# mimoralea/gym-soccer-littman94

Hardware: AMD Instinct MI355X
Metric: env-steps/sec (whole node) at batch=1M random joint actions; HBM GB/s vs peak (higher is better)
Workload: dtype int8

## Files before the change

gym_soccer_littman94_amd/csrc/soccer_handle.hpp:

```cpp
#pragma once
#include <hip/hip_runtime.h>

#include <string>
#include <vector>

#include "../../include/soccer_hip.h"
#include "soccer_inlists.hpp"
#include "soccer_kernels.hpp"
#include "soccer_plan_io.hpp"
#include "soccer_rules.hpp"

#pragma GCC visibility push(hidden)

using namespace soccer;

int fail(soccer_handle* h, int code, const char* fmt, ...);

#define HIP_TRY(h, expr)                                                                         \
    do {                                                                                         \
        hipError_t e_ = (expr);                                                                  \
        if (e_ != hipSuccess)                                                                    \
            return fail((h), e_ == hipErrorOutOfMemory ? SOCCER_E_NOMEM : SOCCER_E_HIP,          \
                        "%s failed: %s", #expr, hipGetErrorString(e_));                          \
    } while (0)

template <typename T>
static inline bool aligned(const T* p, size_t a) { return p == nullptr || (reinterpret_cast<uintptr_t>(p) % a) == 0; }

template <class T> static inline T* off(T* p, unsigned long long lanes) { return p ? p + lanes : nullptr; }

struct OwnedBufs {
    struct Buf { void* ptr; bool pinned; };
    enum PinnedFlags : unsigned { kPinned = hipHostMallocDefault, kPinnedMapped = hipHostMallocMapped };
    const char* what;
    std::vector<Buf> bufs;
    bool ready = false;
    explicit OwnedBufs(const char* owner) : what(owner) {}
    OwnedBufs(const OwnedBufs&) = delete;
    OwnedBufs& operator=(const OwnedBufs&) = delete;
    ~OwnedBufs() { clear(); }

    template <class T>
    int alloc(soccer_handle* h, size_t count, T** out) { return take(h, hipMalloc(out, bytes<T>(count)), false, out); }
    template <class T>
    int alloc_pinned(soccer_handle* h, size_t count, PinnedFlags flags, T** out) { return take(h, hipHostMalloc(out, bytes<T>(count), flags), true, out); }
    template <class T>
    int upload(soccer_handle* h, const std::vector<T>& v, const T** out) {
        T* d = nullptr;
        if (int rc = alloc(h, v.size(), &d)) return rc;
        if (!v.empty() && hipMemcpy(d, v.data(), v.size() * sizeof(T), hipMemcpyHostToDevice) != hipSuccess)
            return fail(h, SOCCER_E_HIP, "upload of %s failed", what);
        *out = d;
        return SOCCER_OK;
    }
    void release(void* p) {
        for (size_t i = 0; i < bufs.size(); ++i) if (bufs[i].ptr == p) { drop(bufs[i]); bufs.erase(bufs.begin() + i); return; }
    }
    void clear() {
        for (const Buf& b : bufs) drop(b);
        bufs.clear(); ready = false;
    }

private:
    template <class T> static size_t bytes(size_t count) { return count ? count * sizeof(T) : 1; }
    static void drop(const Buf& b) { (void)(b.pinned ? hipHostFree(b.ptr) : hipFree(b.ptr)); }
    template <class T>
    int take(soccer_handle* h, hipError_t e, bool pinned, T** out) {
        if (e != hipSuccess) {
            *out = nullptr;
            return e == hipErrorOutOfMemory ? fail(h, SOCCER_E_NOMEM, "out of %s memory for %s", pinned ? "pinned host" : "device", what)
                                            : fail(h, SOCCER_E_HIP, "allocation for %s failed: %s", what, hipGetErrorString(e));
        }
        bufs.push_back(Buf{*out, pinned});
        return SOCCER_OK;
    }
};

struct soccer_graph {
    hipGraph_t graph = nullptr;
    hipGraphExec_t exec = nullptr;
    uint64_t ticks = 0;
    int start_slot = 0;
    bool stamped = false;
    int32_t kernel_nodes = 0;
    int64_t steps_fused = 0;
    int32_t fused_launches = 0;
};

struct PendingRun {
    soccer_step_args first{};
    int64_t len = 0;
    int64_t act_stride = 0, out_stride = 0;
};

struct Learner;

struct soccer_handle {
    soccer_config cfg{};
    Rules rules;
    KernelParams P{};
    hipStream_t stream = nullptr;
    bool own_stream = false;
    hipEvent_t ev0 = nullptr, ev1 = nullptr;
    OwnedBufs bufs{"the handle"};
    uint16_t* d_lut = nullptr; uint32_t* d_nc = nullptr; uint32_t* d_isd = nullptr;
    int8_t* d_policy[2] = {nullptr, nullptr};
    unsigned long long* d_tick = nullptr;
    unsigned long long* d_hist = nullptr;
    unsigned int* d_misuse = nullptr;
    unsigned int* misuse_host = nullptr;
    uint8_t* d_state = nullptr;
    size_t state_stride = 0;
    int state_streams = 6;
    uint8_t* stage_dev = nullptr;
    uint8_t* stage_host = nullptr;
    bool mapped = false;
    size_t stage_bytes = 0;
    int tick_slot = 0;
    uint64_t tick = 0;
    bool slip = false, lut_lds = false;
    size_t smem_bytes = 0;
    int E = 4;
    int grid_cap = 2048;
    bool capturing = false;
    uint64_t capture_ticks = 0;
    int capture_calls = 0;
    int capture_start_slot = 0;
    PendingRun run;
    bool graph_fuse = true;
    int capture_kernels = 0;
    int64_t capture_steps_fused = 0; int capture_fused_launches = 0;
    unsigned long long* d_hist_unread = nullptr;
    int n_cu = 256;
    size_t lds_limit = 64 * 1024;
    uint4* d_sub = nullptr;
    uint4* rec_host = nullptr; uint4* rec_dev = nullptr; uint32_t rec_seq = 0;
    swar::Consts swar_c{}; bool swar_ok = false;
    swar::SlipConsts slip_c{}; bool slip_swar_ok = false;
    uint32_t* d_slip_lut = nullptr;
    uint32_t* d_slip_step_lut = nullptr;
    size_t hist_slots = kHistSlots;
    bool timer_stamped = false; int wall_clock_khz = 100000;
    bool capture_stamped = false;
    bool stamp_poll = false;
    unsigned long long stamp_prev = 0;
    unsigned long long swar_launch_lanes = kSwarLaunchLanes;
    int rollout_pref = 0;
    soccer_rollout_shape_info last_rollout{};
    SlipF64* d_slip_f64 = nullptr;
    uint32_t* d_worklist = nullptr;
    unsigned long long* d_traj_hist = nullptr;
    void* comm = nullptr; int comm_world = 0, comm_rank = 0;
    unsigned long long* d_comm_scratch = nullptr;
    PlanIO plan{};
    OwnedBufs plan_bufs{"the planner lists"};
    MinimaxIO mm{};
    double* mm_V[2] = {nullptr, nullptr};
    unsigned long long* mm_words = nullptr;
    OwnedBufs mm_bufs{"the minimax planner"};
    double* br_pol[2] = {nullptr, nullptr};
    double* br_V[2] = {nullptr, nullptr};
    double* br_Qr = nullptr;
    int32_t* br_arg = nullptr;
    unsigned long long* br_words = nullptr;
    int br_cap = 0; bool br_pairs = false;
    OwnedBufs br_bufs{"the best-response solver"};
    double* cx_pol = nullptr;
    double* cx_V[2] = {nullptr, nullptr};
    unsigned long long* cx_words = nullptr;
    int32_t* cx_done = nullptr;
    int32_t* cx_iter = nullptr;
    double* cx_payoff = nullptr;
    int32_t* cx_open = nullptr;
    double* cx_values = nullptr;
    int cx_policies = 0, cx_stride = 0; bool cx_has_values = false;
    OwnedBufs cx_bufs{"the cross-play solver"};
    double* mo_pol = nullptr;
    double* mo_V[2] = {nullptr, nullptr};
    unsigned long long* mo_words = nullptr;
    int32_t* mo_done = nullptr;
    int32_t* mo_iter = nullptr;
    double* mo_kickoff = nullptr;
    int32_t* mo_open = nullptr;
    double* mo_values = nullptr;
    int mo_policies = 0, mo_stride = 0; bool mo_has_values = false;
    OwnedBufs mo_bufs{"the match-outcome solver"};
    const int32_t* oc_in_offset = nullptr;
    const InEntry* oc_in_list = nullptr;
    OwnedBufs oc_lists{"the occupancy solver's in-lists"};
    double* oc_pol = nullptr;
    double* oc_polT = nullptr;
    double* oc_D[2] = {nullptr, nullptr};
    unsigned long long* oc_words = nullptr;
    int32_t* oc_done = nullptr;
    int32_t* oc_iter = nullptr;
    double* oc_length = nullptr;
    double* oc_expect = nullptr;
    double* oc_features = nullptr;
    int32_t* oc_open = nullptr;
    double* oc_values = nullptr;
    int oc_policies = 0, oc_stride = 0; bool oc_has_values = false;
    OwnedBufs oc_bufs{"the occupancy solver"};
    double* pg_pol = nullptr;
    double* pg_polT = nullptr;
    double* pg_V[2] = {nullptr, nullptr};
    double* pg_D[2] = {nullptr, nullptr};
    double* pg_Q = nullptr;
    unsigned long long* pg_words = nullptr;
    int32_t* pg_done[2] = {nullptr, nullptr};
    int32_t* pg_iter = nullptr;
    double* pg_payoff = nullptr;
    int32_t* pg_open = nullptr;
    double* pg_grad = nullptr;
    double* pg_reach = nullptr;
    double* pg_w = nullptr;
    double* pg_values = nullptr;
    int pg_policies = 0, pg_stride = 0; bool pg_has_values = false;
    OwnedBufs pg_bufs{"the policy-gradient solver"};
    std::vector<soccer_gradient_play*> gradient_players;
    double* mg_A = nullptr;
    double* mg_T = nullptr;
    double* mg_x = nullptr; double* mg_y = nullptr;
    double* mg_fcol = nullptr; double* mg_prow = nullptr;
    int32_t* mg_basis = nullptr;
    double* mg_scal = nullptr;
    int32_t* mg_int = nullptr;
    size_t mg_need[5] = {0, 0, 0, 0, 0};
    OwnedBufs mg_bufs{"the meta-game solver"};
    std::vector<Learner*> learners;
    std::string err;

    soccer_handle() = default;
    soccer_handle(const soccer_handle&) = delete;
    soccer_handle& operator=(const soccer_handle&) = delete;
    ~soccer_handle();
};

constexpr size_t kStampStride = 8;
constexpr size_t kMappedBytes = 64 + 8 * kStampStride * SOCCER_STAMP_SLOTS;

static inline void bind_tick(soccer_handle* h, KernelParams& P, uint64_t ticks) {
    P.tick_in = h->d_tick + (h->tick_slot ? 16 : 0);
    P.tick_out = h->d_tick + (h->tick_slot ? 0 : 16);
    h->tick_slot ^= 1;
    if (h->capturing) { h->capture_ticks += ticks; h->capture_calls += 1; }
    else h->tick += ticks;
}

static inline void note_kernel(soccer_handle* h) { if (h->capturing) h->capture_kernels += 1; }

static inline int grid_for(const soccer_handle* h, uint64_t work_items) {
    uint64_t blocks = (work_items + kBlock - 1) / kBlock;
    if (blocks < 1) blocks = 1;
    if (blocks > (uint64_t)h->grid_cap) blocks = h->grid_cap;
    return static_cast<int>(blocks);
}

hipError_t rollout_raise_smem_limit(const soccer_handle* h, size_t bytes);
bool rollout_takes_swar(const soccer_handle* h, const soccer_rollout_args* a, const soccer_rollout_extra* x);
int rollout_enqueue(soccer_handle* h, const soccer_rollout_args* a, const soccer_rollout_extra* x, unsigned long long* hist);
int flush_run(soccer_handle* h);
static inline int flush_pending(soccer_handle* h) { return h->run.len ? flush_run(h) : SOCCER_OK; }
void comm_release(soccer_handle* h);
void learners_release(soccer_handle* h);
void gradient_players_release(soccer_handle* h);

#pragma GCC visibility pop
```

gym_soccer_littman94_amd/csrc/soccer_hip.hip:

```cpp
#include <hip/hip_runtime.h>

#include <algorithm>
#include <atomic>
#include <chrono>
#include <cstdarg>
#include <cstdio>
#include <cstdlib>
#include <cstring>
#include <memory>
#include <string>
#include <vector>

#include "soccer_handle.hpp"
#include "soccer_env_kernels.hpp"
#include "soccer_slip.hpp"

static thread_local std::string g_err;

int fail(soccer_handle* h, int code, const char* fmt, ...) {
    char buf[512];
    va_list ap; va_start(ap, fmt); vsnprintf(buf, sizeof buf, fmt, ap); va_end(ap);
    if (h) h->err = buf; else g_err = buf;
    return code;
}

extern "C" int soccer_abi_version(void) { return SOCCER_ABI_VERSION; }

extern "C" int soccer_device_count(int* count) {
    if (!count) return fail(nullptr, SOCCER_E_INVALID, "count is NULL");
    HIP_TRY(nullptr, hipGetDeviceCount(count));
    return SOCCER_OK;
}

extern "C" const char* soccer_last_error(const soccer_handle* h) { return h ? h->err.c_str() : g_err.c_str(); }

soccer_handle::~soccer_handle() {
    (void)hipSetDevice(cfg.device);
    (void)hipStreamSynchronize(stream);
    comm_release(this);
    learners_release(this);
    gradient_players_release(this);
    bufs.clear(); plan_bufs.clear(); mm_bufs.clear(); br_bufs.clear();
    if (ev0) (void)hipEventDestroy(ev0);
    if (ev1) (void)hipEventDestroy(ev1);
    if (own_stream && stream) (void)hipStreamDestroy(stream);
}

static void set_key(soccer_handle* h, uint64_t seed) {
    h->cfg.seed = seed;
    h->P.key0 = static_cast<uint32_t>(seed);
    h->P.key1 = static_cast<uint32_t>(seed >> 32);
}

extern "C" int soccer_create(const soccer_config* cfg, soccer_handle** out) {
    if (!cfg || !out) return fail(nullptr, SOCCER_E_INVALID, "cfg/out is NULL");
    *out = nullptr;
    if (cfg->n_lanes < 1) return fail(nullptr, SOCCER_E_INVALID, "n_lanes must be >= 1");
    if (!(cfg->slip_prob >= 0.0 && cfg->slip_prob <= 1.0))
        return fail(nullptr, SOCCER_E_INVALID, "slip_prob must be in [0, 1]");
    if (cfg->max_steps < 1 || cfg->max_steps > 250)
        return fail(nullptr, SOCCER_E_INVALID, "max_steps must be in 1..250 (timestep is a uint8)");
    const uint32_t e = cfg->envs_per_thread;
    if (!(e == 0 || e == 1 || e == 4 || e == 8))
        return fail(nullptr, SOCCER_E_INVALID, "envs_per_thread must be 0, 1, 4 or 8");
    std::unique_ptr<soccer_handle> owner(new soccer_handle());
    soccer_handle* h = owner.get();
    h->cfg = *cfg;
    const std::string msg = h->rules.build(cfg->width, cfg->height);
    if (!msg.empty()) return fail(nullptr, SOCCER_E_INVALID, "%s", msg.c_str());
    int ndev = 0;
    hipError_t de = hipGetDeviceCount(&ndev);
    if (de != hipSuccess || ndev < 1)
        return fail(nullptr, SOCCER_E_HIP, "no HIP device available (%s); libsoccer_hip has no CPU path",
                    de == hipSuccess ? "device count is 0" : hipGetErrorString(de));
    if (cfg->device < 0 || cfg->device >= ndev) return fail(nullptr, SOCCER_E_INVALID, "device %d out of range (0..%d)", cfg->device, ndev - 1);
    HIP_TRY(nullptr, hipSetDevice(cfg->device));
    if (cfg->flags & SOCCER_F_NULL_STREAM) { h->stream = nullptr; h->own_stream = false; }
    else if (cfg->stream) { h->stream = static_cast<hipStream_t>(cfg->stream); h->own_stream = false; }
    else { HIP_TRY(nullptr, hipStreamCreateWithFlags(&h->stream, hipStreamNonBlocking)); h->own_stream = true; }
    HIP_TRY(nullptr, hipEventCreate(&h->ev0));
    HIP_TRY(nullptr, hipEventCreate(&h->ev1));

    const Rules& R = h->rules;
    KernelParams& P = h->P;
    const size_t n = cfg->n_lanes;
    const size_t padded = (n + 255) & ~size_t(255);
    h->state_stride = padded;
    h->mapped = (cfg->flags & SOCCER_F_HOST_MAPPED) != 0;
    if (h->mapped && n > 4096) return fail(nullptr, SOCCER_E_INVALID, "SOCCER_F_HOST_MAPPED is for small handles (n_lanes <= 4096)");
    const char* lay = std::getenv("SOCCER_STATE_LAYOUT");
    const bool packed = swar::packs(R.H, R.W) && !h->mapped && !(lay && std::strcmp(lay, "wide") == 0);
    h->state_streams = packed ? 3 : 6;
    const size_t state_bytes = (size_t)h->state_streams * padded;
    if (int rc = h->mapped ? h->bufs.alloc_pinned(nullptr, state_bytes, OwnedBufs::kPinnedMapped, &h->d_state)
                           : h->bufs.alloc(nullptr, state_bytes, &h->d_state)) return rc;
    P.state = h->d_state; P.state_stride = padded; P.state_layout = packed ? kStatePacked : kStateWide;
    {
        uint8_t init[6] = {(uint8_t)R.isd[0][0], (uint8_t)R.isd[0][1], (uint8_t)R.isd[0][2], (uint8_t)R.isd[0][3], (uint8_t)(2 | R.isd[0][4]), 0};
        if (packed) {
            uint32_t a, b, t;
            swar::pack3(swar::Group{init[0], init[1], init[2], init[3], init[4], init[5]}, a, b, t);
            init[0] = (uint8_t)a; init[1] = (uint8_t)b; init[2] = (uint8_t)t;
        }
        for (int k = 0; k < h->state_streams; ++k) {
            if (h->mapped) std::memset(h->d_state + k * padded, init[k], padded);
            else HIP_TRY(nullptr, hipMemsetAsync(h->d_state + k * padded, init[k], padded, h->stream));
        }
    }

    if (int rc = h->bufs.alloc(nullptr, R.next_cell.size(), &h->d_nc)) return rc;
    if (int rc = h->bufs.alloc(nullptr, sizeof(R.isd_words) / sizeof(uint32_t), &h->d_isd)) return rc;
    HIP_TRY(nullptr, hipMemcpy(h->d_isd, R.isd_words, sizeof(R.isd_words), hipMemcpyHostToDevice));
    HIP_TRY(nullptr, hipMemcpy(h->d_nc, R.next_cell.data(), R.next_cell.size() * sizeof(uint32_t), hipMemcpyHostToDevice));
    if (int rc = h->bufs.alloc(nullptr, 256 / sizeof(unsigned long long), &h->d_tick)) return rc;
    HIP_TRY(nullptr, hipMemset(h->d_tick, 0, 256));
    while (h->hist_slots < (n + 255) / 256) h->hist_slots <<= 1;
    if (int rc = h->bufs.alloc(nullptr, h->hist_slots * kHistStride, &h->d_hist)) return rc;
    HIP_TRY(nullptr, hipMemset(h->d_hist, 0, sizeof(unsigned long long) * h->hist_slots * kHistStride));
    if (int rc = h->bufs.alloc(nullptr, h->hist_slots * kHistStride, &h->d_hist_unread)) return rc;
    HIP_TRY(nullptr, hipMemset(h->d_hist_unread, 0, sizeof(unsigned long long) * h->hist_slots * kHistStride));
    if (int rc = h->bufs.alloc_pinned(nullptr, kMappedBytes / sizeof(unsigned int), OwnedBufs::kPinnedMapped, &h->misuse_host)) return rc;
    std::memset(h->misuse_host, 0, kMappedBytes);
    HIP_TRY(nullptr, hipHostGetDevicePointer(reinterpret_cast<void**>(&h->d_misuse), h->misuse_host, 0));

    P.next_cell = h->d_nc; P.isd = h->d_isd;
    P.hist = h->d_hist; P.hist_mask = (uint32_t)(h->hist_slots - 1); P.misuse = h->d_misuse;
    P.lane_offset = cfg->lane_offset;
    P.first = 0; P.n = n; P.W = R.W; P.HW = R.H * R.W; P.HW5 = 5 * R.H * R.W;
    P.nc_len = static_cast<int32_t>(R.next_cell.size());
    P.max_steps = cfg->max_steps;
    P.autoreset = (cfg->flags & SOCCER_F_AUTORESET) ? 1u : 0u;
    P.step_stats = (cfg->flags & SOCCER_F_STEP_STATS) ? 1u : 0u;
    P.isd_shift = R.n_isd == 4 ? 0u : 1u;
    {
        const SlipTables ST = build_slip_tables(cfg->slip_prob);
        for (int i = 0; i < 4; ++i) P.w[i] = ST.w[i];
        for (int i = 0; i < 9; ++i) { P.B[i] = ST.B[i]; P.CB[i] = ST.CB[i]; }
        P.nb = ST.nb; P.act_pack = ST.act_pack; P.slip_int = ST.slip_int;
        static_assert(sizeof(swar::Quad) == sizeof(uint4), "threshold rows are 16 bytes");
        if (int rc = h->bufs.alloc(nullptr, sizeof(ST.sub) / sizeof(uint4), &h->d_sub)) return rc;
        HIP_TRY(nullptr, hipMemcpy(h->d_sub, ST.sub, sizeof(ST.sub), hipMemcpyHostToDevice));
        P.sub = h->d_sub;
        h->slip_swar_ok = ST.swar_ok;
        static_assert(kSlipBuckets == 16384 && kSlipThresholds == 40, "table layout shared with the kernels");
        if (ST.lut_ok) {
            std::vector<uint32_t> img(kSlipLdsWords, 0xFFFFFFFFu);
            std::memcpy(img.data(), ST.lut, kSlipBuckets);
            std::memcpy(img.data() + kSlipBuckets / 4, ST.T, sizeof(ST.T));
            if (int rc = h->bufs.alloc(nullptr, img.size(), &h->d_slip_lut)) return rc;
            HIP_TRY(nullptr, hipMemcpy(h->d_slip_lut, img.data(), img.size() * sizeof(uint32_t), hipMemcpyHostToDevice));
        }
        if (ST.lut_step_ok && !std::getenv("SOCCER_STEP_SLIP_ONE_BY_ONE")) {
            std::vector<uint32_t> img(kSlipStepLdsWords, 0xFFFFFFFFu);
            std::memcpy(img.data(), ST.lut_step, kSlipStepBuckets);
            std::memcpy(img.data() + kSlipStepBuckets / 4, ST.T, sizeof(ST.T));
            if (int rc = h->bufs.alloc(nullptr, img.size(), &h->d_slip_step_lut)) return rc;
            HIP_TRY(nullptr, hipMemcpy(h->d_slip_step_lut, img.data(), img.size() * sizeof(uint32_t), hipMemcpyHostToDevice));
        }
        {
            const SlipF64 F = make_slip_f64(ST);
            if (int rc = h->bufs.alloc(nullptr, 1, &h->d_slip_f64)) return rc;
            HIP_TRY(nullptr, hipMemcpy(h->d_slip_f64, &F, sizeof F, hipMemcpyHostToDevice));
        }
        h->slip_c = swar::SlipConsts{};
        for (int i = 0; i < 9; ++i) h->slip_c.CB[i] = ST.CB[i];
        h->slip_c.c_off = ST.c_off;
    }
    set_key(h, cfg->seed);
    h->swar_ok = swar::fits(R.H, R.W, cfg->max_steps);
    if (h->swar_ok) h->swar_c = swar::make_consts(R.H, R.W, R.goal_lo, R.goal_hi, cfg->max_steps, R.n_isd, R.isd, P.autoreset != 0u);
    h->slip = cfg->slip_prob != 0.0;
    if (const char* e2 = std::getenv("SOCCER_ROLLOUT")) h->rollout_pref = std::atoi(e2);
    if (const char* e4 = std::getenv("SOCCER_GRAPH_FUSE")) h->graph_fuse = std::atoi(e4) != 0;
    if (const char* e3 = std::getenv("SOCCER_SWAR_LAUNCH_LANES")) {
        const unsigned long long v = std::strtoull(e3, nullptr, 10) & ~3ull;
        if (v >= 4ull && v <= kSwarLaunchLanes) h->swar_launch_lanes = v;
    }
    h->E = e ? static_cast<int>(e) : 4;

    const size_t nc_bytes = (R.next_cell.size() + kIsdWords) * sizeof(uint32_t);
    const size_t lut_bytes = R.lut.size() * sizeof(uint16_t);
    if (nc_bytes > 150 * 1024)
        return fail(nullptr, SOCCER_E_INVALID, "pitch too large: the move/bounds table (%zu bytes) must fit the 160 KB LDS", nc_bytes);
    if (int rc = h->bufs.alloc(nullptr, R.lut.size(), &h->d_lut)) return rc;
    HIP_TRY(nullptr, hipMemcpy(h->d_lut, R.lut.data(), lut_bytes, hipMemcpyHostToDevice));
    P.lut = h->d_lut; P.lut_len = static_cast<int32_t>(R.lut.size());
    h->lut_lds = nc_bytes + lut_bytes <= 150 * 1024;
    h->smem_bytes = nc_bytes + (h->lut_lds ? lut_bytes : 0);
    if (h->smem_bytes > 48 * 1024) {
        const size_t b = h->smem_bytes;
        hipError_t se = rollout_raise_smem_limit(h, b);
        if (se == hipSuccess)
            se = hipFuncSetAttribute(h->slip ? reinterpret_cast<const void*>(h->lut_lds ? &reset_kernel<true, true> : &reset_kernel<false, true>)
                                             : reinterpret_cast<const void*>(h->lut_lds ? &reset_kernel<true, false> : &reset_kernel<false, false>),
                                     hipFuncAttributeMaxDynamicSharedMemorySize, (int)b);
        HIP_TRY(nullptr, se);
    }
    hipDeviceProp_t prop;
    HIP_TRY(nullptr, hipGetDeviceProperties(&prop, cfg->device));
    { int khz = 0; if (hipDeviceGetAttribute(&khz, hipDeviceAttributeWallClockRate, cfg->device) == hipSuccess && khz > 0) h->wall_clock_khz = khz; }
    h->grid_cap = prop.multiProcessorCount * 8;
    h->n_cu = prop.multiProcessorCount;
    if (prop.sharedMemPerBlockOptin > 0) h->lds_limit = prop.sharedMemPerBlockOptin;
    else if (prop.sharedMemPerBlock > 0) h->lds_limit = prop.sharedMemPerBlock;
    HIP_TRY(nullptr, hipStreamSynchronize(h->stream));
    HIP_TRY(nullptr, hipDeviceSynchronize());
    *out = owner.release();
    return SOCCER_OK;
}

extern "C" int soccer_destroy(soccer_handle* h) {
    delete h;
    return SOCCER_OK;
}

extern "C" int soccer_sync(soccer_handle* h) {
    if (!h) return fail(nullptr, SOCCER_E_INVALID, "handle is NULL");
    if (h->capturing) return fail(h, SOCCER_E_STATE, "soccer_sync during graph capture");
    HIP_TRY(h, hipSetDevice(h->cfg.device));
    HIP_TRY(h, hipStreamSynchronize(h->stream));
    return SOCCER_OK;
}

extern "C" int soccer_seed(soccer_handle* h, uint64_t seed) {
    if (!h) return fail(nullptr, SOCCER_E_INVALID, "handle is NULL");
    if (h->capturing) return fail(h, SOCCER_E_STATE, "soccer_seed during graph capture");
    HIP_TRY(h, hipSetDevice(h->cfg.device));
    set_key(h, seed);
    h->tick = 0;
    HIP_TRY(h, hipMemsetAsync(h->d_tick, 0, 256, h->stream));
    return SOCCER_OK;
}

extern "C" uint64_t soccer_tick(const soccer_handle* h) { return h ? h->tick : 0; }

extern "C" int soccer_set_tick(soccer_handle* h, uint64_t tick) {
    if (!h) return fail(nullptr, SOCCER_E_INVALID, "handle is NULL");
    if (h->capturing) return fail(h, SOCCER_E_STATE, "soccer_set_tick during graph capture");
    if (tick >> 63) return fail(h, SOCCER_E_INVALID, "tick must be below 2^63");
    HIP_TRY(h, hipSetDevice(h->cfg.device));
    HIP_TRY(h, hipStreamSynchronize(h->stream));
    unsigned long long slots[32] = {0};
    slots[0] = tick; slots[16] = tick;
    HIP_TRY(h, hipMemcpy(h->d_tick, slots, sizeof slots, hipMemcpyHostToDevice));
    h->tick = tick;
    return SOCCER_OK;
}
extern "C" uint64_t soccer_get_seed(const soccer_handle* h) { return h ? h->cfg.seed : 0; }

extern "C" int batched_reset(soccer_handle* h, const uint8_t* mask, const double* u_reset, uint16_t* obs) {
    if (!h) return fail(nullptr, SOCCER_E_INVALID, "handle is NULL");
    if (!aligned(u_reset, 8) || !aligned(obs, 2))
        return fail(h, SOCCER_E_INVALID, "batched_reset: u_reset must be 8-byte and obs 2-byte aligned");
    HIP_TRY(h, hipSetDevice(h->cfg.device));
    if (int rc = flush_pending(h)) return rc;
    KernelParams P = h->P;
    bind_tick(h, P, 1);
    ResetIO io{mask, u_reset, obs};
    unsigned long long n4 = 0;
    if (h->swar_ok && !u_reset && h->E != 1 && (P.lane_offset & 3ull) == 0ull && aligned(mask, 4) && aligned(obs, 8)) n4 = P.n & ~3ull;
    if (n4) {
        ResetSwar RS{h->swar_c, P.state, P.state_stride, P.state_layout, n4, P.lane_offset, P.tick_in, P.tick_out, P.key0, P.key1, mask, obs};
        const dim3 g(static_cast<unsigned>(((n4 >> 2) + kBlock - 1) / kBlock)), b(kBlock);
        if (h->slip) { if (mask) hipLaunchKernelGGL((reset_kernel_swar<true, true>), g, b, 0, h->stream, RS);
                       else hipLaunchKernelGGL((reset_kernel_swar<false, true>), g, b, 0, h->stream, RS); }
        else { if (mask) hipLaunchKernelGGL((reset_kernel_swar<true, false>), g, b, 0, h->stream, RS);
               else hipLaunchKernelGGL((reset_kernel_swar<false, false>), g, b, 0, h->stream, RS); }
        note_kernel(h);
    }
    if (n4 < P.n) {
        KernelParams Q = P;
        Q.first = n4; Q.n = P.n - n4;
        if (n4) Q.tick_out = nullptr;
        const int grid = grid_for(h, Q.n);
        if (h->slip) { if (h->lut_lds) hipLaunchKernelGGL((reset_kernel<true, true>), dim3(grid), dim3(kBlock), h->smem_bytes, h->stream, Q, io);
                       else hipLaunchKernelGGL((reset_kernel<false, true>), dim3(grid), dim3(kBlock), h->smem_bytes, h->stream, Q, io); }
        else { if (h->lut_lds) hipLaunchKernelGGL((reset_kernel<true, false>), dim3(grid), dim3(kBlock), h->smem_bytes, h->stream, Q, io);
               else hipLaunchKernelGGL((reset_kernel<false, false>), dim3(grid), dim3(kBlock), h->smem_bytes, h->stream, Q, io); }
        note_kernel(h);
    }
    HIP_TRY(h, hipGetLastError());
    return SOCCER_OK;
}

static int fetch_state(soccer_handle* h, std::vector<uint8_t>& img) {
    const size_t n = h->P.n, S = h->state_stride, bytes = (size_t)h->state_streams * S;
    if (h->mapped) std::memcpy(img.data(), h->d_state, bytes);
    else HIP_TRY(h, hipMemcpy(img.data(), h->d_state, bytes, hipMemcpyDeviceToHost));
    if (h->state_streams == 3) {
        for (size_t i = 0; i < n; ++i) {
            swar::Group G;
            swar::unpack3(img[i], img[S + i], img[2 * S + i], G);
            img[5 * S + i] = (uint8_t)G.tt; img[4 * S + i] = (uint8_t)G.ps; img[3 * S + i] = (uint8_t)G.cb;
            img[2 * S + i] = (uint8_t)G.rb; img[S + i] = (uint8_t)G.ca; img[i] = (uint8_t)G.ra;
        }
    }
    return SOCCER_OK;
}

extern "C" int soccer_state_streams(const soccer_handle* h) { return h ? h->state_streams : 0; }

extern "C" int soccer_set_state(soccer_handle* h, const int8_t* row_a, const int8_t* col_a, const int8_t* row_b,
                                const int8_t* col_b, const uint8_t* poss, const uint8_t* t,
                                const uint8_t* needs_reset) {
    if (!h) return fail(nullptr, SOCCER_E_INVALID, "handle is NULL");
    if (h->capturing) return fail(h, SOCCER_E_STATE, "soccer_set_state during graph capture");
    HIP_TRY(h, hipSetDevice(h->cfg.device));
    HIP_TRY(h, hipStreamSynchronize(h->stream));
    const size_t n = h->P.n, S = h->state_stride;
    const Rules& R = h->rules;
    std::vector<uint8_t> img(6 * S);
    if (int rc = fetch_state(h, img)) return rc;
    int8_t* ra = reinterpret_cast<int8_t*>(img.data());
    int8_t* ca = ra + S; int8_t* rb = ra + 2 * S; int8_t* cb = ra + 3 * S;
    uint8_t* ps = img.data() + 4 * S; uint8_t* tt = img.data() + 5 * S;
    for (size_t i = 0; i < n; ++i) {
        if (row_a) ra[i] = row_a[i];
        if (col_a) ca[i] = col_a[i];
        if (row_b) rb[i] = row_b[i];
        if (col_b) cb[i] = col_b[i];
        uint8_t p = ps[i] & 1, nr = (ps[i] >> 1) & 1;
        if (poss) { if (poss[i] > 1) return fail(h, SOCCER_E_INVALID, "lane %zu: possession must be 0 or 1", i); p = poss[i]; }
        if (needs_reset) nr = needs_reset[i] ? 1 : 0;
        ps[i] = static_cast<uint8_t>(p | (nr << 1));
        if (t) { if (t[i] > h->cfg.max_steps) return fail(h, SOCCER_E_INVALID, "lane %zu: timestep %d > max_steps", i, (int)t[i]); tt[i] = t[i]; }
        const bool in_range = ra[i] >= 0 && ra[i] < R.H && rb[i] >= 0 && rb[i] < R.H &&
                              ca[i] >= 0 && ca[i] < R.W && cb[i] >= 0 && cb[i] < R.W;
        if (!in_range || R.kind[R.flat(ra[i], ca[i], rb[i], cb[i], p)] == 0)
            return fail(h, SOCCER_E_INVALID, "lane %zu: state (%d, %d, %d, %d, %d) is not a reachable state tuple",
                        i, (int)ra[i], (int)ca[i], (int)rb[i], (int)cb[i], (int)p);
    }
    if (h->state_streams == 3) {
        for (size_t i = 0; i < n; ++i) {
            uint32_t a, b, t_;
            swar::pack3(swar::Group{(uint8_t)ra[i], (uint8_t)ca[i], (uint8_t)rb[i], (uint8_t)cb[i], ps[i], tt[i]}, a, b, t_);
            img[i] = (uint8_t)a; img[S + i] = (uint8_t)b; img[2 * S + i] = (uint8_t)t_;
        }
    }
    const size_t bytes = (size_t)h->state_streams * S;
    if (h->mapped) std::memcpy(h->d_state, img.data(), bytes);
    else HIP_TRY(h, hipMemcpy(h->d_state, img.data(), bytes, hipMemcpyHostToDevice));
    return SOCCER_OK;
}

extern "C" int soccer_host_view(soccer_handle* h, uint8_t** state, uint64_t* stride) {
    if (!h || !state || !stride) return fail(h, SOCCER_E_INVALID, "handle/state/stride is NULL");
    if (!h->mapped) return fail(h, SOCCER_E_STATE, "soccer_host_view needs a SOCCER_F_HOST_MAPPED handle");
    *state = h->d_state; *stride = h->state_stride;
    return SOCCER_OK;
}

extern "C" int soccer_get_state(soccer_handle* h, int8_t* row_a, int8_t* col_a, int8_t* row_b, int8_t* col_b,
                                uint8_t* poss, uint8_t* t, uint8_t* needs_reset) {
    if (!h) return fail(nullptr, SOCCER_E_INVALID, "handle is NULL");
    if (h->capturing) return fail(h, SOCCER_E_STATE, "soccer_get_state during graph capture");
    HIP_TRY(h, hipSetDevice(h->cfg.device));
    HIP_TRY(h, hipStreamSynchronize(h->stream));
    const size_t n = h->P.n, S = h->state_stride;
    std::vector<uint8_t> img(6 * S);
    if (int rc = fetch_state(h, img)) return rc;
    if (row_a) std::memcpy(row_a, img.data(), n);
    if (col_a) std::memcpy(col_a, img.data() + S, n);
    if (row_b) std::memcpy(row_b, img.data() + 2 * S, n);
    if (col_b) std::memcpy(col_b, img.data() + 3 * S, n);
    if (t) std::memcpy(t, img.data() + 5 * S, n);
    const uint8_t* ps = img.data() + 4 * S;
    for (size_t i = 0; i < n; ++i) {
        if (poss) poss[i] = ps[i] & 1;
        if (needs_reset) needs_reset[i] = (ps[i] >> 1) & 1;
    }
    return SOCCER_OK;
}

namespace {
struct StageLayout {
    size_t act_a, act_b, mask, u_step, u_reset;
    size_t obs, final_obs, reward, term, trunc, code;
    size_t out_begin, total;
};
StageLayout stage_layout(size_t n) {
    auto up = [](size_t x) { return (x + 63) & ~size_t(63); };
    StageLayout L{};
    size_t o = 0;
    L.act_a = o; o = up(o + n);
    L.act_b = o; o = up(o + n);
    L.mask = o; o = up(o + n);
    L.u_step = o; o = up(o + 8 * n);
    L.u_reset = o; o = up(o + 8 * n);
    L.out_begin = o;
    L.obs = o; o = up(o + 2 * n);
    L.final_obs = o; o = up(o + 2 * n);
    L.reward = o; o = up(o + n);
    L.term = o; o = up(o + n);
    L.trunc = o; o = up(o + n);
    L.code = o; o = up(o + n);
    L.total = o;
    return L;
}
int ensure_stage(soccer_handle* h, const StageLayout& L) {
    if (h->stage_bytes >= L.total) return SOCCER_OK;
    uint8_t* host = nullptr; uint8_t* dev = nullptr;
    if (int rc = h->bufs.alloc_pinned(h, L.total, h->mapped ? OwnedBufs::kPinnedMapped : OwnedBufs::kPinned, &host)) return rc;
    if (h->mapped) dev = host;
    else if (int rc = h->bufs.alloc(h, L.total, &dev)) { h->bufs.release(host); return rc; }
    h->stage_host = host; h->stage_dev = dev; h->stage_bytes = L.total;
    return SOCCER_OK;
}
}

extern "C" int soccer_staging(soccer_handle* h, soccer_staging_view* v) {
    if (!h || !v) return fail(h, SOCCER_E_INVALID, "handle/view is NULL");
    HIP_TRY(h, hipSetDevice(h->cfg.device));
    const StageLayout L = stage_layout(h->P.n);
    if (int rc = ensure_stage(h, L)) return rc;
    uint8_t* H = h->stage_host;
    v->act_a = reinterpret_cast<int8_t*>(H + L.act_a); v->act_b = reinterpret_cast<int8_t*>(H + L.act_b);
    v->mask = H + L.mask;
    v->u_step = reinterpret_cast<double*>(H + L.u_step); v->u_reset = reinterpret_cast<double*>(H + L.u_reset);
    v->obs = reinterpret_cast<uint16_t*>(H + L.obs); v->final_obs = reinterpret_cast<uint16_t*>(H + L.final_obs);
    v->reward = reinterpret_cast<int8_t*>(H + L.reward); v->terminated = H + L.term; v->truncated = H + L.trunc;
    v->prob_code = H + L.code;
    return SOCCER_OK;
}

static long first_bad_action(const int8_t* a, size_t n) {
    size_t i = 0;
    for (; i + 8 <= n; i += 8) {
        uint64_t v; std::memcpy(&v, a + i, 8);
        if ((v & 0xF8F8F8F8F8F8F8F8ull) | (((v & 0x0707070707070707ull) + 0x0303030303030303ull) & 0x0808080808080808ull)) break;
    }
    for (; i < n; ++i) if (a[i] < 0 || a[i] > 4) return (long)i;
    return -1;
}

extern "C" int batched_step_staged(soccer_handle* h, uint32_t use) {
    if (!h) return fail(nullptr, SOCCER_E_INVALID, "handle is NULL");
    if (h->capturing) return fail(h, SOCCER_E_STATE, "batched_step_staged during graph capture");
    const bool has_a = use & SOCCER_STAGE_ACT_A, has_b = use & SOCCER_STAGE_ACT_B;
    if ((!has_a && !h->P.policy_a) || (!has_b && !h->P.policy_b))
        return fail(h, SOCCER_E_INVALID, "batched_step: an action stream is required for every player without a fixed policy");
    HIP_TRY(h, hipSetDevice(h->cfg.device));
    const size_t n = h->P.n;
    const StageLayout L = stage_layout(n);
    if (int rc = ensure_stage(h, L)) return rc;
    uint8_t* H = h->stage_host; uint8_t* D = h->stage_dev;
    for (int pl = 0; pl < 2; ++pl) {
        if (!(pl ? has_b : has_a)) continue;
        const long bad = first_bad_action(reinterpret_cast<const int8_t*>(H + (pl ? L.act_b : L.act_a)), n);
        if (bad >= 0) return fail(h, SOCCER_E_INVALID, "batched_step: action of player_%c in lane %ld is %d; actions must be in 0..4",
                                  pl ? 'b' : 'a', bad, (int)reinterpret_cast<const int8_t*>(H + (pl ? L.act_b : L.act_a))[bad]);
    }
    if (!h->mapped) {
        if (has_a && has_b) HIP_TRY(h, hipMemcpyAsync(D + L.act_a, H + L.act_a, L.act_b + n - L.act_a, hipMemcpyHostToDevice, h->stream));
        else if (has_a) HIP_TRY(h, hipMemcpyAsync(D + L.act_a, H + L.act_a, n, hipMemcpyHostToDevice, h->stream));
        else if (has_b) HIP_TRY(h, hipMemcpyAsync(D + L.act_b, H + L.act_b, n, hipMemcpyHostToDevice, h->stream));
        if (use & SOCCER_STAGE_U_STEP) HIP_TRY(h, hipMemcpyAsync(D + L.u_step, H + L.u_step, 8 * n, hipMemcpyHostToDevice, h->stream));
        if (use & SOCCER_STAGE_U_RESET) HIP_TRY(h, hipMemcpyAsync(D + L.u_reset, H + L.u_reset, 8 * n, hipMemcpyHostToDevice, h->stream));
    }
    soccer_step_args d{};
    d.act_a = has_a ? reinterpret_cast<const int8_t*>(D + L.act_a) : nullptr;
    d.act_b = has_b ? reinterpret_cast<const int8_t*>(D + L.act_b) : nullptr;
    d.u_step = (use & SOCCER_STAGE_U_STEP) ? reinterpret_cast<const double*>(D + L.u_step) : nullptr;
    d.u_reset = (use & SOCCER_STAGE_U_RESET) ? reinterpret_cast<const double*>(D + L.u_reset) : nullptr;
    d.obs = reinterpret_cast<uint16_t*>(D + L.obs); d.final_obs = reinterpret_cast<uint16_t*>(D + L.final_obs);
    d.reward = reinterpret_cast<int8_t*>(D + L.reward); d.terminated = D + L.term; d.truncated = D + L.trunc;
    d.prob_code = D + L.code;
    if (int rc = batched_step_ex(h, &d)) return rc;
    if (!h->mapped) HIP_TRY(h, hipMemcpyAsync(H + L.out_begin, D + L.out_begin, L.total - L.out_begin, hipMemcpyDeviceToHost, h->stream));
    HIP_TRY(h, hipStreamSynchronize(h->stream));
    return SOCCER_OK;
}

extern "C" int batched_reset_staged(soccer_handle* h, uint32_t use) {
    if (!h) return fail(nullptr, SOCCER_E_INVALID, "handle is NULL");
    if (h->capturing) return fail(h, SOCCER_E_STATE, "batched_reset_staged during graph capture");
    HIP_TRY(h, hipSetDevice(h->cfg.device));
    const size_t n = h->P.n;
    const StageLayout L = stage_layout(n);
    if (int rc = ensure_stage(h, L)) return rc;
    uint8_t* H = h->stage_host; uint8_t* D = h->stage_dev;
    if (!h->mapped) {
        if (use & SOCCER_STAGE_MASK) HIP_TRY(h, hipMemcpyAsync(D + L.mask, H + L.mask, n, hipMemcpyHostToDevice, h->stream));
        if (use & SOCCER_STAGE_U_RESET) HIP_TRY(h, hipMemcpyAsync(D + L.u_reset, H + L.u_reset, 8 * n, hipMemcpyHostToDevice, h->stream));
    }
    if (int rc = batched_reset(h, (use & SOCCER_STAGE_MASK) ? D + L.mask : nullptr,
                               (use & SOCCER_STAGE_U_RESET) ? reinterpret_cast<const double*>(D + L.u_reset) : nullptr,
                               reinterpret_cast<uint16_t*>(D + L.obs))) return rc;
    if (!h->mapped) HIP_TRY(h, hipMemcpyAsync(H + L.obs, D + L.obs, 2 * n, hipMemcpyDeviceToHost, h->stream));
    HIP_TRY(h, hipStreamSynchronize(h->stream));
    return SOCCER_OK;
}

static int scalar_call(soccer_handle* h, const char* what, uint32_t op, soccer_scalar_io* io) {
    if (!h) return fail(nullptr, SOCCER_E_INVALID, "handle is NULL");
    if (!io) return fail(h, SOCCER_E_INVALID, "%s: io is NULL", what);
    if (h->capturing) return fail(h, SOCCER_E_STATE, "%s during graph capture", what);
    if (h->P.n != 1) return fail(h, SOCCER_E_INVALID, "%s needs a handle with n_lanes == 1", what);
    const Rules& R = h->rules;
    ScalarIO k{};
    k.op = op; k.u_step = io->u_step; k.u_reset = io->u_reset;
    if (op == 0u) {
        if (io->needs_reset) return fail(h, SOCCER_E_INVALID, "Please reset the environment before taking a step");
        const int ra = io->row_a, ca = io->col_a, rb = io->row_b, cb = io->col_b;
        if (ra < 0 || ra >= R.H || rb < 0 || rb >= R.H || ca < 0 || ca >= R.W || cb < 0 || cb >= R.W || io->poss > 1)
            return fail(h, SOCCER_E_INVALID, "%s: tuple (%d, %d, %d, %d, %d) is outside the pitch", what, ra, ca, rb, cb, (int)io->poss);
        if (R.kind[((((size_t)ra * R.W + ca) * R.H + rb) * R.W + cb) * 2 + io->poss] == 0)
            return fail(h, SOCCER_E_INVALID, "%s: tuple (%d, %d, %d, %d, %d) is unreachable", what, ra, ca, rb, cb, (int)io->poss);
        if ((int)io->t > h->cfg.max_steps) return fail(h, SOCCER_E_INVALID, "%s: t = %d exceeds max_steps", what, (int)io->t);
        if ((!h->P.policy_a && (io->act_a < 0 || io->act_a > 4)) || (!h->P.policy_b && (io->act_b < 0 || io->act_b > 4)))
            return fail(h, SOCCER_E_INVALID, "%s: actions must be in 0..4", what);
        k.pos = (uint32_t)ra | ((uint32_t)ca << 8) | ((uint32_t)rb << 16) | ((uint32_t)cb << 24);
        k.misc = (uint32_t)io->poss | ((uint32_t)io->t << 8) | ((uint32_t)(uint8_t)io->act_a << 16) | ((uint32_t)(uint8_t)io->act_b << 24);
    }
    HIP_TRY(h, hipSetDevice(h->cfg.device));
    if (!h->rec_host) {
        uint4* rec = nullptr;
        if (int rc = h->bufs.alloc_pinned(h, 64 / sizeof(uint4), OwnedBufs::kPinnedMapped, &rec)) return rc;
        std::memset(rec, 0, 64);
        const hipError_t e = hipHostGetDevicePointer(reinterpret_cast<void**>(&h->rec_dev), rec, 0);
        if (e != hipSuccess) { h->bufs.release(rec); return fail(h, SOCCER_E_HIP, "%s: no device address for the result record: %s", what, hipGetErrorString(e)); }
        h->rec_host = rec;
    }
    k.seq = ++h->rec_seq ? h->rec_seq : ++h->rec_seq;
    k.record = h->rec_dev;
    KernelParams P = h->P;
    bind_tick(h, P, 1);
    if (h->slip) hipLaunchKernelGGL(scalar_kernel<true>, dim3(1), dim3(64), 0, h->stream, P, k);
    else hipLaunchKernelGGL(scalar_kernel<false>, dim3(1), dim3(64), 0, h->stream, P, k);
    HIP_TRY(h, hipGetLastError());
    volatile uint32_t* flag = reinterpret_cast<volatile uint32_t*>(h->rec_host);
    const auto t_start = std::chrono::steady_clock::now();
    auto byte_sum = [](uint32_t a, uint32_t b) { uint32_t s_ = 0; for (int q = 0; q < 4; ++q) s_ += ((a >> (8 * q)) & 0xffu) + ((b >> (8 * q)) & 0xffu); return s_ & 0xffu; };
    auto landed = [&]() {
        const uint32_t f0 = flag[0], f1 = flag[1], f2 = flag[2], f3 = flag[3];
        return f0 == k.seq && (f3 >> 24) == (k.seq & 0xffu) && ((f3 >> 16) & 0xffu) == byte_sum(f1, f2);
    };
    for (uint32_t spins = 0; !landed(); ++spins) {
        __builtin_ia32_pause();
        if ((spins & 0xfffffu) == 0xfffffu) {
            const hipError_t e = hipStreamQuery(h->stream);
            if (e != hipSuccess && e != hipErrorNotReady) return fail(h, SOCCER_E_HIP, "%s: %s", what, hipGetErrorString(e));
            if (e == hipSuccess && !landed()) return fail(h, SOCCER_E_HIP, "%s: the kernel finished without publishing its record", what);
            if (std::chrono::steady_clock::now() - t_start > std::chrono::seconds(30))
                return fail(h, SOCCER_E_HIP, "%s: no result after 30 s (is another stream hogging the device?)", what);
        }
    }
    std::atomic_thread_fence(std::memory_order_acquire);
    const volatile uint32_t* r = flag;
    const uint32_t res = r[1], npos = r[2], nm = r[3];
    io->obs = (uint16_t)(res & 0xffffu); io->reward = (int8_t)((res >> 16) & 0xffu);
    io->terminated = (res >> 24) & 1u; io->truncated = (res >> 25) & 1u; io->prob_code = (uint8_t)(res >> 26);
    io->row_a = (int8_t)(npos & 0xffu); io->col_a = (int8_t)((npos >> 8) & 0xffu);
    io->row_b = (int8_t)((npos >> 16) & 0xffu); io->col_b = (int8_t)(npos >> 24);
    io->poss = nm & 1u; io->needs_reset = (nm >> 1) & 1u; io->t = (uint8_t)((nm >> 8) & 0xffu);
    return SOCCER_OK;
}

extern "C" int soccer_step_scalar(soccer_handle* h, soccer_scalar_io* io) { return scalar_call(h, "soccer_step_scalar", 0u, io); }
extern "C" int soccer_reset_scalar(soccer_handle* h, soccer_scalar_io* io) { return scalar_call(h, "soccer_reset_scalar", 1u, io); }

extern "C" int batched_step_host(soccer_handle* h, const soccer_step_args* a) {
    if (!h) return fail(nullptr, SOCCER_E_INVALID, "handle is NULL");
    if (!a) return fail(h, SOCCER_E_INVALID, "batched_step: arguments are NULL");
    if (a->last_return || a->reward_a_f32 || a->reward_b_f32 || a->finished)
        return fail(h, SOCCER_E_INVALID, "batched_step_host: last_return / reward_*_f32 / finished are device-only");
    soccer_staging_view v{};
    if (int rc = soccer_staging(h, &v)) return rc;
    const size_t n = h->P.n;
    uint32_t use = 0;
    if (a->act_a) { std::memcpy(v.act_a, a->act_a, n); use |= SOCCER_STAGE_ACT_A; }
    if (a->act_b) { std::memcpy(v.act_b, a->act_b, n); use |= SOCCER_STAGE_ACT_B; }
    if (a->u_step) { std::memcpy(v.u_step, a->u_step, 8 * n); use |= SOCCER_STAGE_U_STEP; }
    if (a->u_reset) { std::memcpy(v.u_reset, a->u_reset, 8 * n); use |= SOCCER_STAGE_U_RESET; }
    if (int rc = batched_step_staged(h, use)) return rc;
    if (a->obs) std::memcpy(a->obs, v.obs, 2 * n);
    if (a->final_obs) std::memcpy(a->final_obs, v.final_obs, 2 * n);
    if (a->reward) std::memcpy(a->reward, v.reward, n);
    if (a->terminated) std::memcpy(a->terminated, v.terminated, n);
    if (a->truncated) std::memcpy(a->truncated, v.truncated, n);
    if (a->prob_code) std::memcpy(a->prob_code, v.prob_code, n);
    return SOCCER_OK;
}

extern "C" int batched_reset_host(soccer_handle* h, const uint8_t* mask, const double* u_reset, uint16_t* obs) {
    if (!h) return fail(nullptr, SOCCER_E_INVALID, "handle is NULL");
    soccer_staging_view v{};
    if (int rc = soccer_staging(h, &v)) return rc;
    const size_t n = h->P.n;
    uint32_t use = 0;
    if (mask) { std::memcpy(v.mask, mask, n); use |= SOCCER_STAGE_MASK; }
    if (u_reset) { std::memcpy(v.u_reset, u_reset, 8 * n); use |= SOCCER_STAGE_U_RESET; }
    if (int rc = batched_reset_staged(h, use)) return rc;
    if (obs) std::memcpy(obs, v.obs, 2 * n);
    return SOCCER_OK;
}


extern "C" int soccer_set_policy(soccer_handle* h, int32_t player, const int8_t* policy_host, int32_t n_states) {
    if (!h) return fail(nullptr, SOCCER_E_INVALID, "handle is NULL");
    if (h->capturing) return fail(h, SOCCER_E_STATE, "soccer_set_policy during graph capture");
    if (player != 0 && player != 1) return fail(h, SOCCER_E_INVALID, "player must be 0 (player_a) or 1 (player_b)");
    HIP_TRY(h, hipSetDevice(h->cfg.device));
    HIP_TRY(h, hipStreamSynchronize(h->stream));
    const int8_t** slot = player == 0 ? &h->P.policy_a : &h->P.policy_b;
    h->plan_bufs.clear();
    if (!policy_host) { *slot = nullptr; return SOCCER_OK; }
    if (n_states != h->rules.nS) return fail(h, SOCCER_E_INVALID, "policy must have one action per observation index (%d)", h->rules.nS);
    if ((player == 0 ? h->P.policy_b : h->P.policy_a) != nullptr)
        return fail(h, SOCCER_E_INVALID, "Both players cannot have a policy. At least one must be None.");
    for (int i = 0; i < n_states; ++i)
        if (policy_host[i] < 0 || policy_host[i] > 4) return fail(h, SOCCER_E_INVALID, "policy[%d] = %d is not an action", i, (int)policy_host[i]);
    if (!h->d_policy[player]) if (int rc = h->bufs.alloc(h, (size_t)h->rules.nS, &h->d_policy[player])) return rc;
    HIP_TRY(h, hipMemcpy(h->d_policy[player], policy_host, (size_t)n_states, hipMemcpyHostToDevice));
    *slot = h->d_policy[player];
    return SOCCER_OK;
}

extern "C" int soccer_dims(const soccer_handle* h, int32_t* n_states, int32_t* lut_len, int32_t* n_isd,
                           int32_t* internal_width) {
    if (!h) return fail(nullptr, SOCCER_E_INVALID, "handle is NULL");
    if (n_states) *n_states = h->rules.nS;
    if (lut_len) *lut_len = static_cast<int32_t>(h->rules.lut.size());
    if (n_isd) *n_isd = h->rules.n_isd;
    if (internal_width) *internal_width = h->rules.W;
    return SOCCER_OK;
}

extern "C" int soccer_get_tables(const soccer_handle* h, uint16_t* lut, int8_t* goal_value, int8_t* isd_states) {
    if (!h) return fail(nullptr, SOCCER_E_INVALID, "handle is NULL");
    const Rules& R = h->rules;
    if (lut) std::memcpy(lut, R.lut.data(), R.lut.size() * sizeof(uint16_t));
    if (goal_value) std::memcpy(goal_value, R.goal_value.data(), R.goal_value.size());
    if (isd_states) for (int i = 0; i < R.n_isd; ++i) for (int k = 0; k < 5; ++k) isd_states[i * 5 + k] = R.isd[i][k];
    return SOCCER_OK;
}

extern "C" int soccer_prob_table(const soccer_handle* h, double prob[12]) {
    if (!h || !prob) return fail(nullptr, SOCCER_E_INVALID, "handle/prob is NULL");
    static const double nsp[3] = {1.0, 0.5, 0.25};
    for (int c = 0; c < 4; ++c) for (int k = 0; k < 3; ++k) prob[c * 3 + k] = h->P.w[c] * nsp[k];
    return SOCCER_OK;
}

extern "C" int soccer_get_stats(soccer_handle* h, uint64_t hist[3], uint64_t* misuse) {
    if (!h) return fail(nullptr, SOCCER_E_INVALID, "handle is NULL");
    if (h->capturing) return fail(h, SOCCER_E_STATE, "soccer_get_stats during graph capture");
    HIP_TRY(h, hipSetDevice(h->cfg.device));
    HIP_TRY(h, hipStreamSynchronize(h->stream));
    if (hist) {
        std::vector<unsigned long long> shards(h->hist_slots * kHistStride);
        HIP_TRY(h, hipMemcpy(shards.data(), h->d_hist, shards.size() * sizeof(unsigned long long), hipMemcpyDeviceToHost));
        hist[0] = hist[1] = hist[2] = 0;
        for (size_t s = 0; s < h->hist_slots; ++s) for (int b = 0; b < 3; ++b) hist[b] += shards[s * kHistStride + b];
    }
    if (misuse) {
        const volatile unsigned int* m = h->misuse_host;
        *misuse = (m[0] ? 1u : 0u) | (m[1] ? 2u : 0u) | (m[2] ? 4u : 0u);
    }
    return SOCCER_OK;
}

extern "C" uint32_t soccer_peek_misuse(const soccer_handle* h) {
    if (!h || !h->misuse_host) return 0u;
    const volatile unsigned int* m = h->misuse_host;
    return (m[0] ? SOCCER_MISUSE_FROZEN : 0u) | (m[1] ? SOCCER_MISUSE_ACTION : 0u) | (m[2] ? SOCCER_MISUSE_OBSERVATION : 0u);
}

extern "C" int soccer_reset_stats(soccer_handle* h) {
    if (!h) return fail(nullptr, SOCCER_E_INVALID, "handle is NULL");
    HIP_TRY(h, hipSetDevice(h->cfg.device));
    if (int rc = flush_pending(h)) return rc;
    HIP_TRY(h, hipMemsetAsync(h->d_hist, 0, sizeof(unsigned long long) * h->hist_slots * kHistStride, h->stream));
    HIP_TRY(h, hipMemsetAsync(h->d_misuse, 0, 64, h->stream));
    return SOCCER_OK;
}

extern "C" int soccer_malloc(soccer_handle* h, size_t bytes, void** dptr) {
    if (!h || !dptr) return fail(h, SOCCER_E_INVALID, "handle/dptr is NULL");
    HIP_TRY(h, hipSetDevice(h->cfg.device));
    HIP_TRY(h, hipMalloc(dptr, bytes ? bytes : 1));
    return SOCCER_OK;
}
extern "C" int soccer_free(soccer_handle* h, void* dptr) {
    if (!h) return fail(nullptr, SOCCER_E_INVALID, "handle is NULL");
    HIP_TRY(h, hipSetDevice(h->cfg.device));
    if (dptr) HIP_TRY(h, hipFree(dptr));
    return SOCCER_OK;
}
extern "C" int soccer_memcpy_h2d(soccer_handle* h, void* dst, const void* src, size_t bytes) {
    if (!h) return fail(nullptr, SOCCER_E_INVALID, "handle is NULL");
    if (h->capturing) return fail(h, SOCCER_E_STATE, "soccer_memcpy_h2d during graph capture");
    HIP_TRY(h, hipSetDevice(h->cfg.device));
    HIP_TRY(h, hipMemcpyAsync(dst, src, bytes, hipMemcpyHostToDevice, h->stream));
    HIP_TRY(h, hipStreamSynchronize(h->stream));
    return SOCCER_OK;
}
extern "C" int soccer_memcpy_d2h(soccer_handle* h, void* dst, const void* src, size_t bytes) {
    if (!h) return fail(nullptr, SOCCER_E_INVALID, "handle is NULL");
    if (h->capturing) return fail(h, SOCCER_E_STATE, "soccer_memcpy_d2h during graph capture");
    HIP_TRY(h, hipSetDevice(h->cfg.device));
    HIP_TRY(h, hipMemcpyAsync(dst, src, bytes, hipMemcpyDeviceToHost, h->stream));
    HIP_TRY(h, hipStreamSynchronize(h->stream));
    return SOCCER_OK;
}
extern "C" int soccer_memset(soccer_handle* h, void* dst, int value, size_t bytes) {
    if (!h) return fail(nullptr, SOCCER_E_INVALID, "handle is NULL");
    HIP_TRY(h, hipSetDevice(h->cfg.device));
    if (int rc = flush_pending(h)) return rc;
    HIP_TRY(h, hipMemsetAsync(dst, value, bytes, h->stream));
    return SOCCER_OK;
}

__global__ void stamp_kernel(unsigned long long* slot) {
    if (threadIdx.x == 0) *slot = wall_clock64();
}

static volatile unsigned long long* stamp_host(soccer_handle* h) {
    return reinterpret_cast<volatile unsigned long long*>(reinterpret_cast<uint8_t*>(h->misuse_host) + 64);
}
static unsigned long long* stamp_dev(soccer_handle* h) {
    return reinterpret_cast<unsigned long long*>(reinterpret_cast<uint8_t*>(h->d_misuse) + 64);
}

extern "C" int soccer_stamp(soccer_handle* h, int32_t slot) {
    if (!h) return fail(nullptr, SOCCER_E_INVALID, "handle is NULL");
    if (slot < 0 || slot >= SOCCER_STAMP_SLOTS) return fail(h, SOCCER_E_INVALID, "stamp slot %d out of range (0..%d)", slot, SOCCER_STAMP_SLOTS - 1);
    HIP_TRY(h, hipSetDevice(h->cfg.device));
    if (int rc = flush_pending(h)) return rc;
    hipLaunchKernelGGL(stamp_kernel, dim3(1), dim3(64), 0, h->stream, stamp_dev(h) + kStampStride * slot);
    HIP_TRY(h, hipGetLastError());
    return SOCCER_OK;
}

extern "C" int soccer_stamps_clear(soccer_handle* h, int32_t first, int32_t count) {
    if (!h) return fail(nullptr, SOCCER_E_INVALID, "handle is NULL");
    if (first < 0 || count < 0 || first + count > SOCCER_STAMP_SLOTS) return fail(h, SOCCER_E_INVALID, "stamp range out of bounds");
    for (int32_t i = 0; i < count; ++i) stamp_host(h)[kStampStride * (first + i)] = 0ull;
    std::atomic_thread_fence(std::memory_order_seq_cst);
    return SOCCER_OK;
}

extern "C" int soccer_stamps_read(soccer_handle* h, int32_t first, int32_t count, uint64_t* ticks, int32_t* khz) {
    if (!h) return fail(nullptr, SOCCER_E_INVALID, "handle is NULL");
    if (first < 0 || count < 0 || first + count > SOCCER_STAMP_SLOTS || (count && !ticks)) return fail(h, SOCCER_E_INVALID, "stamp range out of bounds");
    for (int32_t i = 0; i < count; ++i) ticks[i] = stamp_host(h)[kStampStride * (first + i)];
    if (khz) *khz = h->wall_clock_khz;
    return SOCCER_OK;
}

extern "C" int soccer_timer_start(soccer_handle* h) {
    if (!h) return fail(nullptr, SOCCER_E_INVALID, "handle is NULL");
    HIP_TRY(h, hipSetDevice(h->cfg.device));
    h->timer_stamped = h->capturing;
    if (h->capturing) { h->capture_stamped = true; return soccer_stamp(h, 0); }
    HIP_TRY(h, hipEventRecord(h->ev0, h->stream));
    return SOCCER_OK;
}
extern "C" int soccer_timer_mark(soccer_handle* h) {
    if (!h) return fail(nullptr, SOCCER_E_INVALID, "handle is NULL");
    HIP_TRY(h, hipSetDevice(h->cfg.device));
    if (h->capturing) {
        if (!h->capture_stamped) return fail(h, SOCCER_E_STATE, "soccer_timer_mark in a capture needs soccer_timer_start in the same capture");
        return soccer_stamp(h, 1);
    }
    h->timer_stamped = false;
    HIP_TRY(h, hipEventRecord(h->ev1, h->stream));
    return SOCCER_OK;
}
extern "C" int soccer_timer_read(soccer_handle* h, float* elapsed_ms) {
    if (!h || !elapsed_ms) return fail(h, SOCCER_E_INVALID, "handle/elapsed_ms is NULL");
    if (h->capturing) return fail(h, SOCCER_E_STATE, "soccer_timer_read during graph capture");
    HIP_TRY(h, hipSetDevice(h->cfg.device));
    if (h->timer_stamped) {
        volatile unsigned long long* st = stamp_host(h);
        if (h->stamp_poll) {
            const auto t_start = std::chrono::steady_clock::now();
            for (uint32_t spins = 0; st[kStampStride] == h->stamp_prev; ++spins) {
                __builtin_ia32_pause();
                if ((spins & 0xfffffu) == 0xfffffu) {
                    const hipError_t e = hipStreamQuery(h->stream);
                    if (e != hipSuccess && e != hipErrorNotReady) return fail(h, SOCCER_E_HIP, "soccer_timer_read: %s", hipGetErrorString(e));
                    if (e == hipSuccess && st[kStampStride] == h->stamp_prev) return fail(h, SOCCER_E_STATE, "soccer_timer_read: the stream is idle but the closing stamp was never written");
                    if (std::chrono::steady_clock::now() - t_start > std::chrono::seconds(60))
                        return fail(h, SOCCER_E_HIP, "soccer_timer_read: no closing stamp after 60 s");
                }
            }
            std::atomic_thread_fence(std::memory_order_acquire);
        } else {
            for (uint32_t spins = 0;; ++spins) {
                const hipError_t q = hipStreamQuery(h->stream);
                if (q == hipSuccess) break;
                if (q != hipErrorNotReady) return fail(h, SOCCER_E_HIP, "hipStreamQuery failed: %s", hipGetErrorString(q));
                if (spins > 2000u) { (void)hipGetLastError(); HIP_TRY(h, hipStreamSynchronize(h->stream)); break; }
                __builtin_ia32_pause();
            }
            (void)hipGetLastError();
        }
        *elapsed_ms = (float)((double)(st[kStampStride] - st[0]) / (double)h->wall_clock_khz);
        return SOCCER_OK;
    }
    for (uint32_t spins = 0;; ++spins) {
        const hipError_t q = hipEventQuery(h->ev1);
        if (q == hipSuccess) break;
        if (q != hipErrorNotReady) return fail(h, SOCCER_E_HIP, "hipEventQuery failed: %s", hipGetErrorString(q));
        if (spins > 2000u) { (void)hipGetLastError(); HIP_TRY(h, hipEventSynchronize(h->ev1)); break; }
        __builtin_ia32_pause();
    }
    (void)hipGetLastError();
    HIP_TRY(h, hipEventElapsedTime(elapsed_ms, h->ev0, h->ev1));
    return SOCCER_OK;
}
extern "C" int soccer_timer_stop(soccer_handle* h, float* elapsed_ms) {
    if (int rc = soccer_timer_mark(h)) return rc;
    return soccer_timer_read(h, elapsed_ms);
}

__global__ void move_tick_kernel(unsigned long long* dst, const unsigned long long* src) {
    if (threadIdx.x == 0) *dst = *src;
}

extern "C" int soccer_graph_begin(soccer_handle* h) {
    if (!h) return fail(nullptr, SOCCER_E_INVALID, "handle is NULL");
    if (h->capturing) return fail(h, SOCCER_E_STATE, "graph capture already in progress");
    HIP_TRY(h, hipSetDevice(h->cfg.device));
    HIP_TRY(h, hipStreamBeginCapture(h->stream, hipStreamCaptureModeThreadLocal));
    h->capturing = true; h->capture_ticks = 0; h->capture_calls = 0; h->capture_stamped = false;
    h->capture_start_slot = h->tick_slot;
    h->run = PendingRun{}; h->capture_kernels = 0; h->capture_steps_fused = 0; h->capture_fused_launches = 0;
    return SOCCER_OK;
}

extern "C" int soccer_graph_end(soccer_handle* h, soccer_graph** out) {
    if (!h || !out) return fail(h, SOCCER_E_INVALID, "handle/out is NULL");
    if (!h->capturing) return fail(h, SOCCER_E_STATE, "no graph capture in progress");
    if (const int rc = flush_pending(h)) {
        const std::string why = h->err;
        hipGraph_t dead = nullptr;
        h->capturing = false; h->tick_slot = h->capture_start_slot;
        (void)hipStreamEndCapture(h->stream, &dead);
        if (dead) (void)hipGraphDestroy(dead);
        (void)hipGetLastError();
        h->err = why;
        return rc;
    }
    if (h->capture_calls % 2 != 0) {
        hipLaunchKernelGGL(move_tick_kernel, dim3(1), dim3(64), 0, h->stream,
                           h->d_tick + (h->capture_start_slot ? 16 : 0), h->d_tick + (h->tick_slot ? 16 : 0));
        h->tick_slot = h->capture_start_slot;
    }
    h->capturing = false;
    hipGraph_t graph = nullptr;
    HIP_TRY(h, hipStreamEndCapture(h->stream, &graph));
    soccer_graph* g = new soccer_graph();
    g->kernel_nodes = h->capture_kernels; g->steps_fused = h->capture_steps_fused; g->fused_launches = h->capture_fused_launches;
    g->graph = graph; g->ticks = h->capture_ticks; g->start_slot = h->capture_start_slot; g->stamped = h->capture_stamped;
    hipError_t e = hipGraphInstantiate(&g->exec, graph, nullptr, nullptr, 0);
    if (e != hipSuccess) {
        (void)hipGraphDestroy(graph); delete g;
        return fail(h, SOCCER_E_HIP, "hipGraphInstantiate failed: %s", hipGetErrorString(e));
    }
    (void)hipGraphUpload(g->exec, h->stream);
    (void)hipGetLastError();
    *out = g;
    return SOCCER_OK;
}

extern "C" int soccer_graph_launch(soccer_handle* h, soccer_graph* g, int32_t replays) {
    if (!h || !g) return fail(h, SOCCER_E_INVALID, "handle/graph is NULL");
    if (h->capturing) return fail(h, SOCCER_E_STATE, "soccer_graph_launch during graph capture");
    HIP_TRY(h, hipSetDevice(h->cfg.device));
    if (replays > 0 && h->tick_slot != g->start_slot) {
        HIP_TRY(h, hipMemcpyAsync(h->d_tick + (g->start_slot ? 16 : 0), h->d_tick + (h->tick_slot ? 16 : 0),
                                  sizeof(unsigned long long), hipMemcpyDeviceToDevice, h->stream));
        h->tick_slot = g->start_slot;
    }
    h->stamp_poll = replays == 1 && g->stamped && hipStreamQuery(h->stream) == hipSuccess;
    (void)hipGetLastError();
    h->timer_stamped = g->stamped;
    if (h->stamp_poll) h->stamp_prev = stamp_host(h)[kStampStride];
    for (int32_t r = 0; r < replays; ++r) HIP_TRY(h, hipGraphLaunch(g->exec, h->stream));
    h->tick += g->ticks * (uint64_t)(replays > 0 ? replays : 0);
    return SOCCER_OK;
}

extern "C" int soccer_graph_info(const soccer_graph* g, int32_t* kernel_nodes, int64_t* steps_fused, int32_t* fused_launches) {
    if (!g) return fail(nullptr, SOCCER_E_INVALID, "graph is NULL");
    if (kernel_nodes) *kernel_nodes = g->kernel_nodes;
    if (steps_fused) *steps_fused = g->steps_fused;
    if (fused_launches) *fused_launches = g->fused_launches;
    return SOCCER_OK;
}

extern "C" int soccer_graph_destroy(soccer_handle* h, soccer_graph* g) {
    if (!g) return SOCCER_OK;
    if (h) { (void)hipSetDevice(h->cfg.device); (void)hipStreamSynchronize(h->stream); }
    if (g->exec) (void)hipGraphExecDestroy(g->exec);
    if (g->graph) (void)hipGraphDestroy(g->graph);
    delete g;
    return SOCCER_OK;
}

extern "C" int soccer_trajectory_returns(soccer_handle* h, int32_t n_steps, const int8_t* reward, const uint8_t* terminated,
                                         const uint8_t* truncated, int64_t stride, int8_t* last_return,
                                         int32_t* episode_count, uint64_t hist[3]) {
    if (!h) return fail(nullptr, SOCCER_E_INVALID, "handle is NULL");
    if (h->capturing) return fail(h, SOCCER_E_STATE, "soccer_trajectory_returns during graph capture");
    if (n_steps < 1 || !reward || !terminated || !truncated)
        return fail(h, SOCCER_E_INVALID, "soccer_trajectory_returns: n_steps >= 1 and the reward / terminated / truncated trajectories are required");
    if (stride < (int64_t)h->P.n) return fail(h, SOCCER_E_INVALID, "soccer_trajectory_returns: stride must be >= n_lanes");
    if (!aligned(episode_count, 4)) return fail(h, SOCCER_E_INVALID, "soccer_trajectory_returns: episode_count must be 4-byte aligned");
    HIP_TRY(h, hipSetDevice(h->cfg.device));
    const size_t slots = (size_t)h->grid_cap * 2;
    if (!h->d_traj_hist) if (int rc = h->bufs.alloc(h, slots * 4, &h->d_traj_hist)) return rc;
    const unsigned long long n = h->P.n;
    const bool vec = stride % 4 == 0 && aligned(reward, 4) && aligned(terminated, 4) && aligned(truncated, 4) &&
                     aligned(last_return, 4) && aligned(episode_count, 16);
    const unsigned long long n4 = vec ? (n & ~3ull) : 0ull;
    TrajIO io{reward, terminated, truncated, (long long)stride, n_steps, n4, last_return, episode_count, h->d_traj_hist, 0u};
    uint32_t used = 0;
    if (n4) { used = (uint32_t)grid_for(h, n4 >> 2); hipLaunchKernelGGL(trajectory_returns_kernel<true>, dim3(used), dim3(kBlock), 0, h->stream, io); }
    if (n4 < n) {
        TrajIO t = io;
        t.reward += n4; t.terminated += n4; t.truncated += n4; t.n = n - n4; t.slot0 = used;
        t.last_return = off(last_return, n4); t.episode_count = off(episode_count, n4);
        const uint32_t g2 = (uint32_t)grid_for(h, t.n);
        hipLaunchKernelGGL(trajectory_returns_kernel<false>, dim3(g2), dim3(kBlock), 0, h->stream, t);
        used += g2;
    }
    HIP_TRY(h, hipGetLastError());
    if (hist) {
        std::vector<unsigned long long> part((size_t)used * 4);
        HIP_TRY(h, hipMemcpyAsync(part.data(), h->d_traj_hist, part.size() * sizeof(unsigned long long), hipMemcpyDeviceToHost, h->stream));
        HIP_TRY(h, hipStreamSynchronize(h->stream));
        hist[0] = hist[1] = hist[2] = 0;
        for (uint32_t b = 0; b < used; ++b) for (int k = 0; k < 3; ++k) hist[k] += part[(size_t)b * 4 + k];
    }
    return SOCCER_OK;
}
```

gym_soccer_littman94_amd/csrc/soccer_rollout.hip:

```cpp
#include <hip/hip_runtime.h>

#include <algorithm>

#include "soccer_handle.hpp"
#include "soccer_rollout_kernels.hpp"
#include "soccer_slip.hpp"

static_assert(kSlipLutWords == kSlipLdsWords, "table layout shared with the kernels");

template <int E, bool SLIP, bool LUT_LDS>
static hipError_t raise_smem_limit(size_t bytes) {
    hipError_t e = hipFuncSetAttribute(reinterpret_cast<const void*>(&rollout_kernel<E, SLIP, LUT_LDS, false>),
                                       hipFuncAttributeMaxDynamicSharedMemorySize, (int)bytes);
    if (e != hipSuccess) return e;
    return hipFuncSetAttribute(reinterpret_cast<const void*>(&rollout_kernel<E, SLIP, LUT_LDS, true>),
                               hipFuncAttributeMaxDynamicSharedMemorySize, (int)bytes);
}

hipError_t rollout_raise_smem_limit(const soccer_handle* h, size_t bytes) {
    hipError_t se = hipSuccess;
#define RAISE(EV) if (se == hipSuccess) { se = h->slip ? (h->lut_lds ? raise_smem_limit<EV, true, true>(bytes) : raise_smem_limit<EV, true, false>(bytes)) \
                                                       : (h->lut_lds ? raise_smem_limit<EV, false, true>(bytes) : raise_smem_limit<EV, false, false>(bytes)); }
    RAISE(1) RAISE(4) RAISE(8)
#undef RAISE
    return se;
}

template <int E, bool DYN>
static void launch_rollout2(soccer_handle* h, const KernelParams& P, const RolloutIO& io) {
    const int grid = grid_for(h, (P.n + E - 1) / E);
    const dim3 g(grid), b(kBlock);
    if (h->slip) {
        if (h->lut_lds) hipLaunchKernelGGL((rollout_kernel<E, true, true, DYN>), g, b, h->smem_bytes, h->stream, P, io);
        else hipLaunchKernelGGL((rollout_kernel<E, true, false, DYN>), g, b, h->smem_bytes, h->stream, P, io);
    } else {
        if (h->lut_lds) hipLaunchKernelGGL((rollout_kernel<E, false, true, DYN>), g, b, h->smem_bytes, h->stream, P, io);
        else hipLaunchKernelGGL((rollout_kernel<E, false, false, DYN>), g, b, h->smem_bytes, h->stream, P, io);
    }
    note_kernel(h);
}
template <int E>
static void launch_rollout(soccer_handle* h, const KernelParams& P, const RolloutIO& io) {
    const bool dyn = io.sample_actions || P.policy_a || P.policy_b;
    if (dyn) launch_rollout2<E, true>(h, P, io); else launch_rollout2<E, false>(h, P, io);
}

extern "C" int batched_rollout(soccer_handle* h, const soccer_rollout_args* a) { return batched_rollout_ex(h, a, nullptr); }

extern "C" int soccer_rollout_shape(const soccer_handle* h, soccer_rollout_shape_info* out) {
    if (!h || !out) return SOCCER_E_INVALID;
    *out = h->last_rollout;
    out->lds_limit = h->lds_limit;
    return SOCCER_OK;
}

static bool rollout_vec_ok(const soccer_rollout_args* a, const soccer_rollout_extra* x, int e) {
    const uint16_t* x_fin = x ? x->final_obs : nullptr; const uint8_t* x_code = x ? x->prob_code : nullptr;
    const bool any_out = a->obs || a->reward || a->terminated || a->truncated || x_fin || x_code;
    const bool strides = (a->sample_actions || a->act_stride % e == 0) && (!any_out || a->out_stride % e == 0);
    return strides && aligned(a->act_a, e) && aligned(a->act_b, e) && aligned(a->reward, e) &&
           aligned(a->terminated, e) && aligned(a->truncated, e) && aligned(a->obs, 2 * e) && aligned(x_code, e) && aligned(x_fin, 2 * e) &&
           aligned(a->return_sum, 4 * e) && aligned(a->episode_count, 4 * e);
}

bool rollout_takes_swar(const soccer_handle* h, const soccer_rollout_args* a, const soccer_rollout_extra* x) {
    return h->swar_ok && (!h->slip || h->slip_swar_ok) && h->P.n >= 4ull && ((h->P.lane_offset + h->P.first) & 3ull) == 0ull &&
           rollout_vec_ok(a, x, 4) && h->rollout_pref != 1;
}

extern "C" int batched_rollout_ex(soccer_handle* h, const soccer_rollout_args* a, const soccer_rollout_extra* x) {
    if (!h) return fail(nullptr, SOCCER_E_INVALID, "handle is NULL");
    if (int rc = flush_pending(h)) return rc;
    if (!a || a->n_steps < 1) return fail(h, SOCCER_E_INVALID, "batched_rollout: n_steps must be >= 1");
    if (!a->sample_actions && ((!a->act_a && !h->P.policy_a) || (!a->act_b && !h->P.policy_b)))
        return fail(h, SOCCER_E_INVALID, "batched_rollout: an action stream is required for every player without a fixed policy (or sample_actions)");
    if (!a->sample_actions && a->act_stride < (int64_t)h->P.n)
        return fail(h, SOCCER_E_INVALID, "batched_rollout: act_stride must be >= n_lanes");
    uint16_t* x_fin = x ? x->final_obs : nullptr; uint8_t* x_code = x ? x->prob_code : nullptr;
    const bool any_out = a->obs || a->reward || a->terminated || a->truncated || x_fin || x_code;
    if (!aligned(x_fin, 2)) return fail(h, SOCCER_E_INVALID, "batched_rollout_ex: final_obs must be 2-byte aligned");
    if (any_out && a->out_stride < (int64_t)h->P.n)
        return fail(h, SOCCER_E_INVALID, "batched_rollout: out_stride must be >= n_lanes");
    if (!aligned(a->obs, 2) || !aligned(a->return_sum, 4) || !aligned(a->episode_count, 4) ||
        !aligned(a->mix_a, 8) || !aligned(a->mix_b, 8))
        return fail(h, SOCCER_E_INVALID, "batched_rollout: misaligned obs/return_sum/episode_count/mix_*");
    HIP_TRY(h, hipSetDevice(h->cfg.device));
    return rollout_enqueue(h, a, x, h->P.hist);
}

int rollout_enqueue(soccer_handle* h, const soccer_rollout_args* a, const soccer_rollout_extra* x, unsigned long long* hist) {
    uint16_t* x_fin = x ? x->final_obs : nullptr; uint8_t* x_code = x ? x->prob_code : nullptr;
    int E = h->E;
    while (E > 1 && !rollout_vec_ok(a, x, E)) E = E == 4 ? 1 : E / 2;
    const bool swar_roll = rollout_takes_swar(h, a, x);
    constexpr int kChunk = 4096;
    const Rules& R0 = h->rules;
    for (int s0 = 0; s0 < a->n_steps; s0 += kChunk) {
        const int ns = a->n_steps - s0 < kChunk ? a->n_steps - s0 : kChunk;
        KernelParams P = h->P;
        P.hist = hist;
        bind_tick(h, P, (uint64_t)ns);
        const long long ao = (long long)s0 * a->act_stride, oo = (long long)s0 * a->out_stride;
        RolloutIO io{ns, a->sample_actions, a->mix_a, a->mix_b, a->act_a ? a->act_a + ao : nullptr, a->act_b ? a->act_b + ao : nullptr,
                     (long long)a->act_stride, a->obs ? a->obs + oo : nullptr, a->reward ? a->reward + oo : nullptr,
                     a->terminated ? a->terminated + oo : nullptr, a->truncated ? a->truncated + oo : nullptr,
                     (long long)a->out_stride, a->return_sum, a->episode_count, x_fin ? x_fin + oo : nullptr, x_code ? x_code + oo : nullptr};
        const unsigned long long n_all = P.n, n4 = swar_roll ? (P.n & ~3ull) : 0ull;
        if (swar_roll) {
            P.n = n4;
            const bool dyn = io.sample_actions || P.policy_a || P.policy_b;
            RolloutSwar RS{P.state, P.state_stride, P.state_layout, P.first, P.n, P.lane_offset, P.tick_in, P.tick_out, P.hist, P.misuse,
                           P.policy_a, P.policy_b, P.key0, P.key1,
                           h->swar_c, h->slip_c, reinterpret_cast<const swar::Quad*>(P.sub), P.hist_mask, R0.nS, 0, 0u, 0u, h->d_slip_lut};
            const int sm = !h->slip ? 0 : (h->d_slip_lut ? 2 : 1);
            size_t smem = 36 * sizeof(uint32_t);
            RS.tab_off = (uint32_t)(smem / sizeof(uint32_t));
            const bool fixed = P.policy_a || P.policy_b;
            const size_t staging = io.sample_actions ? 0 : 16 * kBlock * sizeof(uint32_t) + 16;
            const size_t lds_cap = h->lds_limit > staging + (sm == 2 ? kSlipLutWords * sizeof(uint32_t) : 0)
                                 ? h->lds_limit - staging - (sm == 2 ? kSlipLutWords * sizeof(uint32_t) : 0) : 0;
            const bool both_mix = dyn && !fixed && io.sample_actions && io.mix_a && io.mix_b &&
                                  smem + (size_t)R0.nS * sizeof(uint4) <= lds_cap;
            if (both_mix) { RS.lds_tables = 1; smem += (size_t)R0.nS * sizeof(uint4); }
            else if (dyn && (io.mix_a || io.mix_b || fixed)) {
                const size_t need = smem + 2 * (size_t)R0.nS * sizeof(uint2) + 2 * (((size_t)R0.nS + 15) & ~size_t(15));
                if (need <= lds_cap) { RS.lds_tables = 1; smem = need; }
            }
            if (!io.sample_actions) {
                smem = (smem + 15) & ~size_t(15);
                RS.act_off = (uint32_t)(smem / sizeof(uint32_t));
                smem += 16 * kBlock * sizeof(uint32_t);
            }
            const RolloutSwar RS0 = RS; const RolloutIO io0 = io;
            soccer_rollout_shape_info sh{};
            sh.kernel = SOCCER_ROLLOUT_BYTE_PARALLEL; sh.tail = n4 < n_all; sh.slip_selection = sm; sh.small_pitch = h->swar_c.small ? 1 : 0;
            sh.full = (io.final_obs || io.prob_code) ? 1 : 0; sh.dynamic_lds_bytes = smem;
            sh.table_placement = !(dyn && (io.mix_a || io.mix_b || fixed)) ? SOCCER_TABLES_NONE : RS.lds_tables ? SOCCER_TABLES_LDS : SOCCER_TABLES_GLOBAL;
            for (unsigned long long c0 = 0; c0 < n4; c0 += h->swar_launch_lanes) {
            const unsigned long long cn = std::min<unsigned long long>(h->swar_launch_lanes, n4 - c0);
            RS = RS0; io = io0;
            RS.state = RS0.state + P.first + c0; RS.first = 0ull; RS.n = cn; RS.lane_offset = RS0.lane_offset + P.first + c0;
            if (c0 + cn < n4) RS.tick_out = nullptr;
            const unsigned long long lane0 = P.first + c0;
            io.act_a = off(io0.act_a, lane0); io.act_b = off(io0.act_b, lane0); io.obs = off(io0.obs, lane0); io.reward = off(io0.reward, lane0);
            io.terminated = off(io0.terminated, lane0); io.truncated = off(io0.truncated, lane0);
            io.return_sum = off(io0.return_sum, lane0); io.episode_count = off(io0.episode_count, lane0);
            io.final_obs = off(io0.final_obs, lane0); io.prob_code = off(io0.prob_code, lane0);
            const uint64_t groups = cn >> 2;
            uint64_t blocks = (groups + kBlock - 1) / kBlock;
            if (blocks > (uint64_t)h->grid_cap) blocks = h->grid_cap;
            const dim3 g((unsigned)blocks), bl(kBlock);
#define LAUNCH_F(DV, SV, GV, FV) do { if (smem > 48 * 1024) HIP_TRY(h, hipFuncSetAttribute(reinterpret_cast<const void*>(&rollout_swar_kernel<DV, SV, GV, FV>), hipFuncAttributeMaxDynamicSharedMemorySize, (int)smem)); \
                                      hipLaunchKernelGGL((rollout_swar_kernel<DV, SV, GV, FV>), g, bl, smem, h->stream, RS, io); } while (0)
#define LAUNCH_G(DV, SV, GV) do { if (io.final_obs || io.prob_code) LAUNCH_F(DV, SV, GV, true); else LAUNCH_F(DV, SV, GV, false); } while (0)
#define LAUNCH_S(DV, SV) do { if (h->swar_c.small) LAUNCH_G(DV, SV, 1); else LAUNCH_G(DV, SV, 0); } while (0)
            const int dm = !dyn ? 0 : (!fixed && io.sample_actions && !io.mix_a && !io.mix_b) ? 1
                                : both_mix ? 2
                                : (!io.sample_actions && P.policy_a && !P.policy_b && io.act_b) ? 4
                                : (!io.sample_actions && P.policy_b && !P.policy_a && io.act_a) ? 5 : 3;
#define LAUNCH_D(SV) do { if (dm == 0) LAUNCH_S(0, SV); else if (dm == 1) LAUNCH_S(1, SV); else if (dm == 2) LAUNCH_S(2, SV); \
                          else if (dm == 4) LAUNCH_S(4, SV); else if (dm == 5) LAUNCH_S(5, SV); else LAUNCH_S(3, SV); } while (0)
            if (sm == 0) LAUNCH_D(0); else if (sm == 1) LAUNCH_D(1); else LAUNCH_D(2);
            note_kernel(h);
            sh.action_source = dm; sh.parts += 1;
#undef LAUNCH_D
#undef LAUNCH_S
#undef LAUNCH_G
#undef LAUNCH_F
            }
            if (n4 < n_all) {
                KernelParams Q = h->P;
                Q.hist = hist;
                Q.tick_in = P.tick_in; Q.tick_out = nullptr;
                Q.first = n4; Q.n = n_all - n4;
                launch_rollout<1>(h, Q, io0);
            }
            h->last_rollout = sh;
        } else {
            switch (E) {
                case 8: launch_rollout<8>(h, P, io); break;
                case 4: launch_rollout<4>(h, P, io); break;
                default: launch_rollout<1>(h, P, io); break;
            }
            const bool tables = P.policy_a || P.policy_b || (io.sample_actions && (io.mix_a || io.mix_b));
            soccer_rollout_shape_info sh{};
            sh.kernel = SOCCER_ROLLOUT_PER_LANE; sh.action_source = (io.sample_actions || P.policy_a || P.policy_b) ? 3 : 0;
            sh.slip_selection = h->slip ? 1 : 0; sh.full = (io.final_obs || io.prob_code) ? 1 : 0;
            sh.table_placement = tables ? SOCCER_TABLES_GLOBAL : SOCCER_TABLES_NONE; sh.parts = 1; sh.dynamic_lds_bytes = h->smem_bytes;
            h->last_rollout = sh;
        }
        h->last_rollout.chunks = (a->n_steps + kChunk - 1) / kChunk;
        HIP_TRY(h, hipGetLastError());
    }
    return SOCCER_OK;
}
```

gym_soccer_littman94_amd/csrc/soccer_rollout_kernels.hpp:

```cpp
#pragma once
#include "soccer_kernels.hpp"

namespace soccer {

template <int E, bool SLIP, bool DYN>
__device__ __forceinline__ void rollout_group(const Tables& T, const KernelParams& P, const RolloutIO& IO,
                                              unsigned long long i0, unsigned long long tick0,
                                              HistAcc<false>& hist, bool& any_misuse) {
    LaneVec<E> S; S.load(P, i0);
    int32_t ret[E], eps[E];
    uint32_t nonzero = 0u;
#pragma unroll
    for (int j = 0; j < E; ++j) { ret[j] = 0; eps[j] = 0; }
    PackB<E> aa, ab; aa.clear(); ab.clear();
    const bool sample = DYN && IO.sample_actions;
    uint32_t bad_act = 0u;
    if (!sample) {
        if (!DYN || IO.act_a) aa.load_nt(IO.act_a, i0);
        if (!DYN || IO.act_b) ab.load_nt(IO.act_b, i0);
        bad_act |= canon_pack(aa) | canon_pack(ab);
    }
    const bool fixed = DYN && (P.policy_a != nullptr || P.policy_b != nullptr ||
                               (sample && (IO.mix_a != nullptr || IO.mix_b != nullptr)));
    uint32_t s_now[E];
#pragma unroll
    for (int j = 0; j < E; ++j) s_now[j] = fixed ? obs_of(T, P, S.L[j].A, S.L[j].B, S.L[j].p) : 0u;
    for (int s = 0; s < IO.n_steps; ++s) {
        const unsigned long long tick = tick0 + (unsigned long long)s;
        PackB<E> naa = aa, nab = ab;
        if (!sample && s + 1 < IO.n_steps) {
            if (!DYN || IO.act_a) naa.load_nt(IO.act_a + (long long)(s + 1) * IO.act_stride, i0);
            if (!DYN || IO.act_b) nab.load_nt(IO.act_b + (long long)(s + 1) * IO.act_stride, i0);
            bad_act |= canon_pack(naa) | canon_pack(nab);
        }
        uint32_t words[E], awords[E];
        lane_words<E>(P, P.lane_offset + i0, block_tick<SLIP>(tick), 0u, words);
        if (sample) lane_words<E>(P, P.lane_offset + i0, tick, 1u, awords);
        PackB<E> o_rew, o_term, o_trunc, o_code; PackH<E> o_obs, o_fin;
        o_rew.clear(); o_term.clear(); o_trunc.clear(); o_obs.clear(); o_code.clear(); o_fin.clear();
#pragma unroll
        for (int j = 0; j < E; ++j) {
            const Draw d = draw_from_word<SLIP>(words[j], tick);
            uint32_t a = aa.get(j), b = ab.get(j);
            if (sample) {
                const uint32_t ha = awords[j] & 0x7fffu, hb = (awords[j] >> 16) & 0x7fffu;
                a = (ha * 5u) >> 15;
                b = (hb * 5u) >> 15;
                if (IO.mix_a) {
                    const uint2 th = *reinterpret_cast<const uint2*>(IO.mix_a + 4u * s_now[j]);
                    a = (ha >= (th.x & 0xffffu)) + (ha >= (th.x >> 16)) + (ha >= (th.y & 0xffffu)) + (ha >= (th.y >> 16));
                }
                if (IO.mix_b) {
                    const uint2 th = *reinterpret_cast<const uint2*>(IO.mix_b + 4u * s_now[j]);
                    b = (hb >= (th.x & 0xffffu)) + (hb >= (th.x >> 16)) + (hb >= (th.y & 0xffffu)) + (hb >= (th.y >> 16));
                }
            }
            if (fixed) {
                if (P.policy_a) a = (uint32_t)(uint8_t)P.policy_a[s_now[j]];
                if (P.policy_b) b = (uint32_t)(uint8_t)P.policy_b[s_now[j]];
            }
            StepResult R;
            any_misuse |= lane_step<SLIP, true>(T, P, S.L[j], a, b, d, R);
            if (DYN) s_now[j] = R.obs;
            o_obs.put(j, R.obs); o_rew.put(j, (uint32_t)R.reward & 0xffu); o_term.put(j, R.term); o_trunc.put(j, R.trunc);
            o_fin.put(j, R.final_obs); o_code.put(j, R.code);
            ret[j] += R.reward; eps[j] += (int32_t)R.finished; nonzero += (uint32_t)R.reward & 1u;
        }
        const long long off = (long long)s * IO.out_stride;
        if (IO.obs) o_obs.store_nt(IO.obs + off, i0);
        if (IO.reward) o_rew.store_nt(IO.reward + off, i0);
        if (IO.terminated) o_term.store_nt(IO.terminated + off, i0);
        if (IO.truncated) o_trunc.store_nt(IO.truncated + off, i0);
        if (IO.final_obs) o_fin.store_nt(IO.final_obs + off, i0);
        if (IO.prob_code) o_code.store_nt(IO.prob_code + off, i0);
        aa = naa; ab = nab;
    }
    S.store(P, i0);
    {
        int32_t rsum = 0; uint32_t fsum = 0u;
#pragma unroll
        for (int j = 0; j < E; ++j) { rsum += ret[j]; fsum += (uint32_t)eps[j]; }
        hist.add_totals(fsum, rsum, nonzero);
    }
    if (IO.return_sum) add_words<E>(IO.return_sum, i0, ret);
    if (IO.episode_count) add_words<E>(IO.episode_count, i0, eps);
    if (bad_act) P.misuse[1] = 1u;
}

template <int E, bool SLIP, bool LUT_LDS, bool DYN>
__global__ __launch_bounds__(kBlock) void rollout_kernel(const KernelParams P, const RolloutIO IO) {
    extern __shared__ __attribute__((aligned(16))) uint32_t smem[];
    HistAcc<false> hist; hist.init(P);
    const Tables T = stage_tables<LUT_LDS>(P, smem);
    const unsigned long long tick0 = *P.tick_in;
    if (P.tick_out) publish_tick(P, tick0, (unsigned long long)IO.n_steps);
    const unsigned long long groups = (P.n + E - 1) / E;
    bool any_misuse = false;
    for (unsigned long long g = (unsigned long long)blockIdx.x * kBlock + threadIdx.x; g < groups;
         g += (unsigned long long)gridDim.x * kBlock) {
        const unsigned long long rel = g * E, i0 = P.first + rel;
        if (E == 1 || rel + E <= P.n) {
            rollout_group<E, SLIP, DYN>(T, P, IO, i0, tick0, hist, any_misuse);
        } else {
            for (unsigned long long i = rel; i < P.n; ++i)
                rollout_group<1, SLIP, DYN>(T, P, IO, P.first + i, tick0, hist, any_misuse);
        }
    }
    if (any_misuse) P.misuse[0] = 1u;
    hist.flush(P);
}

struct RolloutSwar {
    uint8_t* state; unsigned long long state_stride; uint32_t layout;
    unsigned long long first, n, lane_offset;
    const unsigned long long* tick_in; unsigned long long* tick_out;
    unsigned long long* hist; unsigned int* misuse;
    const int8_t* policy_a; const int8_t* policy_b;
    uint32_t key0, key1;
    swar::Consts C; swar::SlipConsts L; const swar::Quad* sub;
    uint32_t hist_mask;
    int32_t nS; int32_t lds_tables;
    uint32_t act_off;
    uint32_t tab_off;
    const uint32_t* slip_lut;
};

struct SlipSrc { const swar::Quad* sub; const uint8_t* lut; const uint32_t* T; };
constexpr int kSlipLutWords = 4096 + 40;

__device__ __forceinline__ uint32_t count8_le15(uint32_t hs, uint32_t tx, uint32_t ty) {
    typedef unsigned short u16x2 __attribute__((ext_vector_type(2)));
    const uint32_t x = __builtin_bit_cast(uint32_t, __builtin_bit_cast(u16x2, hs) - __builtin_bit_cast(u16x2, tx));
    const uint32_t y = __builtin_bit_cast(uint32_t, __builtin_bit_cast(u16x2, hs) - __builtin_bit_cast(u16x2, ty));
    return (uint32_t)__builtin_popcount(swar::perm(y, x, 0x0b0a0908u));
}
__device__ __forceinline__ uint32_t draw_a15(uint32_t wm) { return swar::perm(0u, wm, 0x01000100u); }
__device__ __forceinline__ uint32_t draw_b15(uint32_t wm) { return swar::perm(0u, wm, 0x03020302u); }

template <int DYNM, int SLIPM, bool GENERAL, int GEO, bool FULL = false>
__device__ __forceinline__ void rollout_swar_group(const RolloutSwar& R, const RolloutIO& IO, const SlipSrc& slip,
                                                   const uint2* mix_a_in, const uint2* mix_b_in, const int8_t* pol_a_in, const int8_t* pol_b_in,
                                                   uint32_t* act_lds,
                                                   uint32_t i0, unsigned long long tick0, swar::Group& S,
                                                   uint32_t& fin_tot, uint32_t& nz_tot, uint32_t& neg_tot,
                                                   uint32_t (&acc)[4], uint32_t& frozen_any, uint32_t& bad_any) {
    constexpr bool DYN = DYNM != 0;
    constexpr bool SLIP = SLIPM != 0;
    constexpr bool STAGED = DYNM == 0 || DYNM == 4 || DYNM == 5;
    constexpr bool TRUSTED = DYNM == 1 || DYNM == 2;
    const bool sample = DYNM == 1 || DYNM == 2 || (DYNM == 3 && IO.sample_actions);
    const uint4* mix_ab = DYNM == 2 ? reinterpret_cast<const uint4*>(mix_a_in) : nullptr;
    const uint2* mix_a = DYNM == 3 ? mix_a_in : nullptr;
    const uint2* mix_b = DYNM == 3 ? mix_b_in : nullptr;
    const int8_t* pol_a = DYNM == 3 || DYNM == 4 ? pol_a_in : nullptr;
    const int8_t* pol_b = DYNM == 3 || DYNM == 5 ? pol_b_in : nullptr;
    const bool use_pol_a = DYNM == 4 || (DYNM == 3 && pol_a != nullptr), use_pol_b = DYNM == 5 || (DYNM == 3 && pol_b != nullptr);
    const bool use_mix_a = DYNM == 3 && sample && mix_a != nullptr;
    const bool use_mix_b = DYNM == 3 && sample && mix_b != nullptr;
    const bool load_a = DYNM == 0 || DYNM == 5 || (DYNM == 3 && !sample && IO.act_a != nullptr);
    const bool load_b = DYNM == 0 || DYNM == 4 || (DYNM == 3 && !sample && IO.act_b != nullptr);
    const bool lane_acc = IO.return_sum != nullptr || IO.episode_count != nullptr;
    const bool by_obs = DYNM == 2 || DYNM == 4 || DYNM == 5 || (DYNM == 3 && (use_pol_a || use_pol_b || use_mix_a || use_mix_b));
    uint32_t aa = 0u, ab = 0u;
    uint32_t nx[16];
#pragma unroll
    for (int k = 0; k < 16; ++k) nx[k] = 0u;
    auto fetch = [&](int sb) {
        uint32_t f0 = i0; asm volatile("" : "+v"(f0));
#pragma unroll
        for (int k = 0; k < 8; ++k) {
            int st = sb + k; st = st < 0 ? 0 : st; st = st < IO.n_steps ? st : IO.n_steps - 1;
            typedef const uint8_t __attribute__((address_space(1)))* gbytes;
            typedef const uint32_t __attribute__((address_space(1)))* gwords;
            gbytes row_a = (gbytes)(IO.act_a + (long long)st * IO.act_stride);
            gbytes row_b = (gbytes)(IO.act_b + (long long)st * IO.act_stride);
            asm volatile("" : "+s"(row_a)); asm volatile("" : "+s"(row_b));
            if (load_a) nx[2 * k] = *(gwords)(row_a + f0);
            if (load_b) nx[2 * k + 1] = *(gwords)(row_b + f0);
        }
    };
    if (STAGED) fetch(-(int)((uint32_t)tick0 & 7u));
    else {
        if (load_a) aa = *reinterpret_cast<const uint32_t*>(IO.act_a + i0);
        if (load_b) ab = *reinterpret_cast<const uint32_t*>(IO.act_b + i0);
    }
    uint32_t s_lo = 0u, s_hi = 0u;
    if (by_obs) {
        const uint32_t cc0 = swar::bfi(swar::mask_of(S.ps << 7), S.cb, S.ca);
        swar::obs4<true>(R.C, S.ra, S.ca, S.rb, S.cb, S.ps & swar::K01, swar::is_zero(cc0) | swar::is_zero(cc0 ^ R.C.Wm1x4), s_lo, s_hi);
    }
    const swar::Consts& C = R.C;
    const unsigned long long q = (R.lane_offset + i0) >> 2;
    uint32_t fin_loc = 0u, nz_loc = 0u, neg_loc = 0u;
    uint32_t p0 = 0u, p1 = 0u, p2 = 0u, p3 = 0u;
    if (!SLIP) {
        const unsigned long long bt = tick0 >> 3;
        const Philox4 b = philox4x32_10((uint32_t)q, (uint32_t)(q >> 32), (uint32_t)bt, (uint32_t)(bt >> 32), R.key0, R.key1);
        swar::transpose4(b.w[0], b.w[1], b.w[2], b.w[3], p0, p1, p2, p3);
        for (uint32_t r = ((uint32_t)tick0 & 7u) >> 1; r != 0u; --r) { p0 = p1; p1 = p2; p2 = p3; }
    }
    for (int s = 0; s < IO.n_steps; ++s) {
        const unsigned long long tick = tick0 + (unsigned long long)s;
        const uint32_t t = (uint32_t)tick & 7u;
        const bool new_block = t == 0u || s == 0;
        uint32_t naa = aa, nab = ab;
        if (STAGED) {
            if (new_block) {
#pragma unroll
                for (int k = 0; k < 16; ++k) if ((k & 1) ? load_b : load_a) act_lds[k * kBlock] = nx[k];
                if (s + 8 - (int)t < IO.n_steps) fetch(s + 8 - (int)t);
            }
            if (load_a) aa = act_lds[(2u * t) * kBlock];
            if (load_b) ab = act_lds[(2u * t + 1u) * kBlock];
        } else if (s + 1 < IO.n_steps) {
            if (load_a) naa = *reinterpret_cast<const uint32_t*>(IO.act_a + (long long)(s + 1) * IO.act_stride + i0);
            if (load_b) nab = *reinterpret_cast<const uint32_t*>(IO.act_b + (long long)(s + 1) * IO.act_stride + i0);
        }
        uint32_t a4 = aa, b4 = ab;
        if (DYN) {
            uint32_t aw[4] = {0u, 0u, 0u, 0u};
            if (sample) {
                const Philox4 ab_blk = philox4x32_10((uint32_t)q, (uint32_t)(q >> 32), (uint32_t)tick, (uint32_t)(tick >> 32) | 0x80000000u, R.key0, R.key1);
                aw[0] = ab_blk.w[0]; aw[1] = ab_blk.w[1]; aw[2] = ab_blk.w[2]; aw[3] = ab_blk.w[3];
                a4 = 0u; b4 = 0u;
            }
#pragma unroll
            for (int j = 0; j < 4; ++j) {
                const uint32_t ob = ((j & 2 ? s_hi : s_lo) >> (16 * (j & 1))) & 0xffffu;
                if (DYNM == 2) {
                    const uint4 th = mix_ab[ob];
                    const uint32_t wm = aw[j] | 0x80008000u;
                    a4 |= count8_le15(draw_a15(wm), th.x, th.y) << (8 * j);
                    b4 |= count8_le15(draw_b15(wm), th.z, th.w) << (8 * j);
                } else if (sample) {
                    const uint32_t ha = aw[j] & 0x7fffu, hb = (aw[j] >> 16) & 0x7fffu;
                    uint32_t a = (ha * 5u) >> 15, b = (hb * 5u) >> 15;
                    const uint32_t wm = aw[j] | 0x80008000u;
                    if (use_mix_a) { const uint2 th = mix_a[ob]; a = count8_le15(draw_a15(wm), th.x, th.y) >> 3; }
                    if (use_mix_b) { const uint2 th = mix_b[ob]; b = count8_le15(draw_b15(wm), th.x, th.y) >> 3; }
                    a4 |= a << (8 * j); b4 |= b << (8 * j);
                }
                if (use_pol_a) a4 = (a4 & ~(0xffu << (8 * j))) | ((uint32_t)(uint8_t)pol_a[ob] << (8 * j));
                if (use_pol_b) b4 = (b4 & ~(0xffu << (8 * j))) | ((uint32_t)(uint8_t)pol_b[ob] << (8 * j));
            }
            if (DYNM == 2) { a4 >>= 3; b4 >>= 3; }
        }
        swar::Out o;
        uint32_t sa = 0u, sb = 0u, cls4 = 0u;
        swar::Rand4 rnd;
        if (SLIP) {
            const Philox4 blk = philox4x32_10((uint32_t)q, (uint32_t)(q >> 32), (uint32_t)tick, (uint32_t)(tick >> 32), R.key0, R.key1);
            uint32_t k4 = 0u;
            const uint32_t ca4 = TRUSTED ? a4 : swar::canon4(a4), cb4 = TRUSTED ? b4 : swar::canon4(b4);
            if (SLIPM == 2) swar::slip_select4_lut(slip.lut, slip.T, R.L.c_off, ca4, cb4, blk.w[0], blk.w[1], blk.w[2], blk.w[3], sa, sb, k4, cls4);
            else swar::slip_select4(R.L, slip.sub, ca4, cb4, blk.w[0], blk.w[1], blk.w[2], blk.w[3], sa, sb, k4, cls4);
            rnd = swar::Rand4{k4 << 6, swar::pack_byte0(blk.w[0], blk.w[1], blk.w[2], blk.w[3]) >> C.isd_shift};
        } else {
            if (t == 0u && s != 0) {
                const unsigned long long bt = tick >> 3;
                uint32_t k0 = R.key0, k1 = R.key1; asm volatile("" : "+s"(k0), "+s"(k1));
                const Philox4 b = philox4x32_10((uint32_t)q, (uint32_t)(q >> 32), (uint32_t)bt, (uint32_t)(bt >> 32), k0, k1);
                swar::transpose4(b.w[0], b.w[1], b.w[2], b.w[3], p0, p1, p2, p3);
            }
            rnd = swar::rand_pair(C.isd_shift, t, p0);
            if (t & 1u) { asm volatile(""); p0 = p1; p1 = p2; p2 = p3; }
        }
        swar::step4<GENERAL, FULL, SLIP, GEO, TRUSTED>(C, S, a4, b4, sa, sb, cls4, rnd, o);
        s_lo = o.obs_lo; s_hi = o.obs_hi;
        const long long row = (long long)s * IO.out_stride;
        uint32_t j0 = i0; asm volatile("" : "+v"(j0));
        if (IO.obs) __builtin_nontemporal_store((unsigned long long)o.obs_lo | ((unsigned long long)o.obs_hi << 32),
                                                reinterpret_cast<unsigned long long*>(reinterpret_cast<uint8_t*>(IO.obs + row) + (j0 << 1)));
        if (IO.reward) __builtin_nontemporal_store(o.rew, reinterpret_cast<uint32_t*>(reinterpret_cast<uint8_t*>(IO.reward + row) + j0));
        if (IO.terminated) __builtin_nontemporal_store(o.term, reinterpret_cast<uint32_t*>(reinterpret_cast<uint8_t*>(IO.terminated + row) + j0));
        if (IO.truncated) __builtin_nontemporal_store(o.trunc, reinterpret_cast<uint32_t*>(reinterpret_cast<uint8_t*>(IO.truncated + row) + j0));
        if (FULL) {
            if (IO.final_obs) __builtin_nontemporal_store((unsigned long long)o.fin_lo | ((unsigned long long)o.fin_hi << 32),
                                                          reinterpret_cast<unsigned long long*>(reinterpret_cast<uint8_t*>(IO.final_obs + row) + (j0 << 1)));
            if (IO.prob_code) __builtin_nontemporal_store(o.code, reinterpret_cast<uint32_t*>(reinterpret_cast<uint8_t*>(IO.prob_code + row) + j0));
        }
        fin_loc += (uint32_t)__builtin_popcount(o.finished & swar::K80);
        if (GENERAL) { nz_loc += (uint32_t)__builtin_popcount(o.rew & swar::K01); neg_loc += (uint32_t)__builtin_popcount(o.rew & swar::K80); }
        else {
            nz_loc += (uint32_t)__builtin_popcount(o.term); neg_loc += (uint32_t)__builtin_popcount(o.rew);
        }
        if (lane_acc) {
            acc[0] = swar::pk_add(acc[0], swar::perm(o.rew << 8, o.rew, 0x08010a00u));
            acc[1] = swar::pk_add(acc[1], swar::perm(o.rew << 8, o.rew, 0x09030b02u));
            const uint32_t f01 = swar::one_of(o.finished);
            acc[2] += swar::perm(0u, f01, 0x0c010c00u); acc[3] += swar::perm(0u, f01, 0x0c030c02u);
        }
        if (GENERAL) frozen_any |= o.frozen;
        if (!TRUSTED) bad_any |= o.bad_action;
        if (!STAGED) { aa = naa; ab = nab; }
    }
    fin_tot += fin_loc; nz_tot += nz_loc;
    neg_tot += GENERAL ? neg_loc : (neg_loc - nz_loc) / 7u;
}

template <int DYNM, int SLIPM, int GEO = 0, bool FULL = false>
__global__ __launch_bounds__(kBlock) void rollout_swar_kernel(const RolloutSwar R, const RolloutIO IO) {
    constexpr bool SLIP = SLIPM != 0;
    constexpr bool DYN = DYNM >= 2;
    extern __shared__ __attribute__((aligned(16))) uint32_t smem[];
    HistAcc<false> hist; hist.init_at(R.hist, R.hist_mask);
    SlipSrc slip{R.sub, nullptr, nullptr};
    const uint2* mix_a = reinterpret_cast<const uint2*>(IO.mix_a);
    const uint2* mix_b = reinterpret_cast<const uint2*>(IO.mix_b);
    const int8_t* pol_a = DYNM == 3 || DYNM == 4 ? R.policy_a : nullptr; const int8_t* pol_b = DYNM == 3 || DYNM == 5 ? R.policy_b : nullptr;
    const bool sample = DYNM == 2 || (DYNM == 3 && IO.sample_actions);
    if (SLIP || (DYN && R.lds_tables)) {
        if (SLIPM == 1) { if (threadIdx.x < 36) smem[threadIdx.x] = reinterpret_cast<const uint32_t*>(R.sub)[threadIdx.x];
                          slip.sub = reinterpret_cast<const swar::Quad*>(smem); }
        if (SLIPM == 2) {
            __shared__ __attribute__((aligned(16))) uint32_t s_slip[SLIPM == 2 ? kSlipLutWords : 4];
            for (int i = threadIdx.x; i < kSlipLutWords; i += kBlock) s_slip[i] = R.slip_lut[i];
            slip.lut = reinterpret_cast<const uint8_t*>(s_slip); slip.T = s_slip + kSlipLutWords - 40;
        }
        if (DYNM == 2) {
            uint4* lab = reinterpret_cast<uint4*>(smem + R.tab_off);
            for (int i = threadIdx.x; i < R.nS; i += kBlock) { const uint2 xa = mix_a[i], xb = mix_b[i]; lab[i] = make_uint4(xa.x, xa.y, xb.x, xb.y); }
            mix_a = reinterpret_cast<const uint2*>(lab); mix_b = nullptr;
        } else if (DYN && R.lds_tables) {
            uint2* la = reinterpret_cast<uint2*>(smem + R.tab_off); uint2* lb = la + R.nS;
            int8_t* pa = reinterpret_cast<int8_t*>(lb + R.nS); int8_t* pb = pa + ((R.nS + 15) & ~15);
            if (sample && mix_a) { for (int i = threadIdx.x; i < R.nS; i += kBlock) la[i] = mix_a[i]; mix_a = la; }
            if (sample && mix_b) { for (int i = threadIdx.x; i < R.nS; i += kBlock) lb[i] = mix_b[i]; mix_b = lb; }
            if (pol_a) { for (int i = threadIdx.x; i < R.nS; i += kBlock) pa[i] = pol_a[i]; pol_a = pa; }
            if (pol_b) { for (int i = threadIdx.x; i < R.nS; i += kBlock) pb[i] = pol_b[i]; pol_b = pb; }
        }
        __syncthreads();
    }
    const unsigned long long tick0 = *R.tick_in;
    if (R.tick_out && blockIdx.x == 0 && threadIdx.x == 0) *R.tick_out = tick0 + (unsigned long long)IO.n_steps;
    const unsigned long long groups = R.n >> 2;
    uint32_t frozen_any = 0u, bad_any = 0u;
    uint32_t* act_lds = smem + R.act_off + threadIdx.x;
    for (unsigned long long g = (unsigned long long)blockIdx.x * kBlock + threadIdx.x; g < groups;
         g += (unsigned long long)gridDim.x * kBlock) {
        const uint32_t i0 = (uint32_t)R.first + ((uint32_t)g << 2);
        const uint8_t* sp = R.state + i0;
        swar::Group S;
        if (R.layout == kStatePacked) {
            swar::unpack3(*reinterpret_cast<const uint32_t*>(sp), *reinterpret_cast<const uint32_t*>(sp + R.state_stride),
                          *reinterpret_cast<const uint32_t*>(sp + 2 * R.state_stride), S);
        } else {
        S.ra = *reinterpret_cast<const uint32_t*>(sp); S.ca = *reinterpret_cast<const uint32_t*>(sp + R.state_stride);
        S.rb = *reinterpret_cast<const uint32_t*>(sp + 2 * R.state_stride); S.cb = *reinterpret_cast<const uint32_t*>(sp + 3 * R.state_stride);
        S.ps = *reinterpret_cast<const uint32_t*>(sp + 4 * R.state_stride); S.tt = *reinterpret_cast<const uint32_t*>(sp + 5 * R.state_stride);
        }
        uint32_t fin_tot = 0u, nz_tot = 0u, neg_tot = 0u;
        uint32_t acc[4] = {0u, 0u, 0u, 0u};
        const uint32_t edge = swar::is_zero(S.ca) | swar::is_zero(S.cb) | swar::is_zero(S.ca ^ R.C.Wm1x4) | swar::is_zero(S.cb ^ R.C.Wm1x4);
        const bool special = R.C.autoreset == 0u || (((S.ps << 6) | edge) & swar::K80) != 0u;
        if (special) rollout_swar_group<DYNM, SLIPM, true, GEO, FULL>(R, IO, slip, mix_a, mix_b, pol_a, pol_b, act_lds, i0, tick0, S, fin_tot, nz_tot, neg_tot, acc, frozen_any, bad_any);
        else rollout_swar_group<DYNM, SLIPM, false, GEO, FULL>(R, IO, slip, mix_a, mix_b, pol_a, pol_b, act_lds, i0, tick0, S, fin_tot, nz_tot, neg_tot, acc, frozen_any, bad_any);
        uint8_t* sw = R.state + i0;
        if (R.layout == kStatePacked) {
            uint32_t pa, pb, pt;
            swar::pack3(S, pa, pb, pt);
            *reinterpret_cast<uint32_t*>(sw) = pa; *reinterpret_cast<uint32_t*>(sw + R.state_stride) = pb; *reinterpret_cast<uint32_t*>(sw + 2 * R.state_stride) = pt;
        } else {
        *reinterpret_cast<uint32_t*>(sw) = S.ra; *reinterpret_cast<uint32_t*>(sw + R.state_stride) = S.ca;
        *reinterpret_cast<uint32_t*>(sw + 2 * R.state_stride) = S.rb; *reinterpret_cast<uint32_t*>(sw + 3 * R.state_stride) = S.cb;
        *reinterpret_cast<uint32_t*>(sw + 4 * R.state_stride) = S.ps; *reinterpret_cast<uint32_t*>(sw + 5 * R.state_stride) = S.tt;
        }
        hist.add_totals(fin_tot, (int32_t)nz_tot - 2 * (int32_t)neg_tot, nz_tot);
        if (IO.return_sum != nullptr || IO.episode_count != nullptr) {
            int32_t ret[4] = {(int32_t)(int16_t)(acc[0] & 0xffffu), (int32_t)(int16_t)(acc[0] >> 16), (int32_t)(int16_t)(acc[1] & 0xffffu), (int32_t)(int16_t)(acc[1] >> 16)};
            int32_t eps[4] = {(int32_t)(acc[2] & 0xffffu), (int32_t)(acc[2] >> 16), (int32_t)(acc[3] & 0xffffu), (int32_t)(acc[3] >> 16)};
            if (IO.return_sum) add_words<4>(IO.return_sum, i0, ret);
            if (IO.episode_count) add_words<4>(IO.episode_count, i0, eps);
        }
    }
    if (frozen_any) R.misuse[0] = 1u;
    if (bad_any) R.misuse[1] = 1u;
    hist.flush_at(R.hist, R.hist_mask);
}

}
```

gym_soccer_littman94_amd/csrc/soccer_step.hip:

```cpp
#include <hip/hip_runtime.h>

#include <algorithm>

#include "soccer_handle.hpp"
#include "soccer_step_kernels.hpp"

static inline size_t worklist_count_word(const soccer_handle* h) { return ((size_t)(h->P.n >> 2) + 5) & ~(size_t)1; }
static inline uint32_t* worklist_count(const soccer_handle* h) { return h->d_worklist ? h->d_worklist + worklist_count_word(h) : nullptr; }
static bool ensure_worklist(soccer_handle* h) {
    if (h->d_worklist) return true;
    const size_t words = worklist_count_word(h) + 2 + 4;
    if (h->bufs.alloc(h, words, &h->d_worklist) != SOCCER_OK) { (void)hipGetLastError(); return false; }
    if (hipMemsetAsync(h->d_worklist, 0, words * sizeof(uint32_t), h->stream) != hipSuccess) {
        (void)hipGetLastError(); h->bufs.release(h->d_worklist); h->d_worklist = nullptr; return false;
    }
    return true;
}

template <bool EXPLICIT_U, bool VEC, bool SHARED>
static void launch_step3(soccer_handle* h, const KernelParams& P, const StepIO& io) {
    const int grid = grid_for(h, (P.n + 3) / 4);
    const dim3 g(grid), b(kBlock);
    if (h->slip) hipLaunchKernelGGL((step_kernel<true, EXPLICIT_U, VEC, SHARED>), g, b, 0, h->stream, P, io);
    else hipLaunchKernelGGL((step_kernel<false, EXPLICIT_U, VEC, SHARED>), g, b, 0, h->stream, P, io);
    note_kernel(h);
}
static void launch_step(soccer_handle* h, const KernelParams& P, const StepIO& io, bool explicit_u, bool vec) {
    const bool shared = ((P.lane_offset + P.first) & 3ull) == 0ull;
    const bool policy_only = explicit_u && !io.u_step && !io.u_reset;
    const bool swar_fit = vec && shared && h->swar_ok && (!h->slip || h->slip_swar_ok) && aligned(io.last_return, 4);
    const bool expl = explicit_u && !policy_only && !h->slip && aligned(io.u_step, 16) && aligned(io.u_reset, 16);
    const bool expl_slip = explicit_u && !policy_only && h->slip && io.u_step && aligned(io.u_step, 16) && aligned(io.u_reset, 16) &&
                           vec && shared && h->swar_ok && aligned(io.last_return, 4) && (P.n >> 2) < 0xffffffffull &&
                           (h->d_worklist || (!h->capturing && ensure_worklist(h)));
    if (((policy_only || !explicit_u || expl) && swar_fit) || expl_slip) {
        const int out = (io.prob_code || io.final_obs || P.step_stats) ? 2
                      : (io.reward_a_f32 || io.reward_b_f32 || io.finished || io.last_return) ? 1 : 0;
        const dim3 b(kBlock);
        const unsigned long long act_stream = (h->cfg.flags & SOCCER_F_STREAM_ACTIONS) ? 1ull : 0ull;
#define SWAR_ARGS P.state + c0, P.state_stride, off(io.act_a, c0), off(io.act_b, c0), (h->capturing ? P.tick_in : nullptr), cn | act_stream, (unsigned long long)(h->tick - 1), Q
#define SWAR_GO(OV, SV, PV, XV) do { if (P.state_layout == kStateWide) hipLaunchKernelGGL((step_kernel_swar<OV, SV, PV, 0, XV, kStateWide>), gh, b, 0, h->stream, SWAR_ARGS); \
                                     else if (h->swar_c.small) hipLaunchKernelGGL((step_kernel_swar<OV, SV, PV, 1, XV, kStatePacked>), gh, b, 0, h->stream, SWAR_ARGS); \
                                     else hipLaunchKernelGGL((step_kernel_swar<OV, SV, PV, 0, XV, kStatePacked>), gh, b, 0, h->stream, SWAR_ARGS); } while (0)
#define SWAR_SLIP(OV, PV) do { if (expl_slip) SWAR_GO(OV, 3, PV, true); else if (expl) SWAR_GO(OV, 0, PV, true); else if (!h->slip) SWAR_GO(OV, 0, PV, false); \
                               else if (h->d_slip_step_lut) SWAR_GO(OV, 2, PV, false); else SWAR_GO(OV, 1, PV, false); } while (0)
#define SWAR_OUT(PV) do { if (out == 2) SWAR_SLIP(2, PV); else if (out == 1) SWAR_SLIP(1, PV); else SWAR_SLIP(0, PV); } while (0)
        for (unsigned long long c0 = P.first; c0 < P.first + P.n; c0 += h->swar_launch_lanes) {
            const unsigned long long cn = std::min<unsigned long long>(h->swar_launch_lanes, P.first + P.n - c0);
            const bool last = c0 + cn == P.first + P.n;
            const dim3 gh(static_cast<unsigned>(((cn >> 2) + kBlock - 1) / kBlock));
            SwarParams Q{h->swar_c, P.key0, P.key1, P.lane_offset + c0, last ? P.tick_out : nullptr, P.misuse,
                         off(io.obs, c0), off(io.reward, c0), off(io.terminated, c0), off(io.truncated, c0),
                         off(io.reward_a_f32, c0), off(io.reward_b_f32, c0), off(io.finished, c0), off(io.last_return, c0),
                         off(io.prob_code, c0), off(io.final_obs, c0),
                         P.step_stats ? P.hist : nullptr, P.hist_mask,
                         h->slip_c, reinterpret_cast<const swar::Quad*>(P.sub), h->d_slip_step_lut,
                         P.policy_a, P.policy_b, off(io.u_step, c0), off(io.u_reset, c0),
                         h->d_slip_f64, h->d_worklist, worklist_count(h)};
            if (P.policy_a || P.policy_b) SWAR_OUT(true); else SWAR_OUT(false);
            note_kernel(h);
            if (expl_slip) {
                KernelParams R = P; R.first = c0; R.n = cn; R.tick_out = nullptr;
                StepIO jo = io; jo.worklist = h->d_worklist; jo.work_count = worklist_count(h);
                hipLaunchKernelGGL((step_kernel<true, true, true, true>), dim3(1), dim3(kBlock), 0, h->stream, R, jo);
                note_kernel(h);
            }
        }
#undef SWAR_OUT
#undef SWAR_SLIP
#undef SWAR_GO
#undef SWAR_ARGS
    } else if (explicit_u) {
        if (vec && shared) launch_step3<true, true, true>(h, P, io); else launch_step3<true, false, false>(h, P, io);
    } else if (vec && shared) {
        const bool lean = !io.prob_code && !io.final_obs && !io.last_return && !io.reward_a_f32 && !io.reward_b_f32 && !io.finished && !P.step_stats;
        const int grid = grid_for(h, (P.n + 3) / 4);
        const dim3 g(grid), b(kBlock);
        if (lean) {
            const unsigned long long blocks = ((P.n >> 2) + kBlock - 1) / kBlock;
            const dim3 gh(static_cast<unsigned>(blocks));
#define HOT_ARGS P.state, P.state_stride, io.act_a, io.act_b, (h->capturing ? P.tick_in : nullptr), P.n, (unsigned long long)(h->tick - 1), P, io
            if (h->slip && P.slip_int == 1u) hipLaunchKernelGGL((step_kernel_hot<true, true>), gh, b, 0, h->stream, HOT_ARGS);
            else if (h->slip) hipLaunchKernelGGL(step_kernel_hot<true>, gh, b, 0, h->stream, HOT_ARGS);
            else hipLaunchKernelGGL(step_kernel_hot<false>, gh, b, 0, h->stream, HOT_ARGS);
            note_kernel(h);
#undef HOT_ARGS
        } else launch_step3<false, true, true>(h, P, io);
    }
    else if (vec) launch_step3<false, true, false>(h, P, io);
    else launch_step3<false, false, false>(h, P, io);
}

static int launch_one_step(soccer_handle* h, const soccer_step_args* a) {
    const bool vec = h->E != 1 && aligned(a->act_a, 4) && aligned(a->act_b, 4) && aligned(a->reward, 4) &&
                     aligned(a->terminated, 4) && aligned(a->truncated, 4) && aligned(a->prob_code, 4) &&
                     aligned(a->obs, 8) && aligned(a->final_obs, 8) && aligned(a->reward_a_f32, 16) && aligned(a->reward_b_f32, 16) &&
                     aligned(a->finished, 4);
    const bool explicit_u = a->u_step || a->u_reset || h->P.policy_a || h->P.policy_b;
    KernelParams P = h->P;
    bind_tick(h, P, 1);
    StepIO io{a->act_a, a->act_b, a->u_step, a->u_reset, a->obs, a->reward, a->terminated, a->truncated,
              a->prob_code, a->final_obs, a->last_return, a->reward_a_f32, a->reward_b_f32, a->finished, nullptr, nullptr};
    const unsigned long long n = h->P.n, n4 = vec ? (n & ~3ull) : 0ull;
    if (n4) { P.first = 0; P.n = n4; launch_step(h, P, io, explicit_u, true); }
    if (n4 < n) {
        KernelParams Q = P;
        Q.first = n4; Q.n = n - n4;
        if (n4) Q.tick_out = nullptr;
        launch_step(h, Q, io, explicit_u, false);
    }
    HIP_TRY(h, hipGetLastError());
    return SOCCER_OK;
}

static soccer_rollout_args run_as_rollout(const soccer_step_args& f, int64_t len, int64_t act_stride, int64_t out_stride) {
    soccer_rollout_args r{};
    r.n_steps = (int32_t)len; r.sample_actions = 0;
    r.act_a = f.act_a; r.act_b = f.act_b; r.act_stride = act_stride;
    r.obs = f.obs; r.reward = f.reward; r.terminated = f.terminated; r.truncated = f.truncated; r.out_stride = out_stride;
    return r;
}

static bool step_can_fuse(const soccer_handle* h, const soccer_step_args* a) {
    if (!h->graph_fuse || !h->own_stream || h->P.policy_a || h->P.policy_b || h->E == 1 || (h->P.n & 3ull)) return false;
    if (a->u_step || a->u_reset || a->reward_a_f32 || a->reward_b_f32 || a->finished || a->last_return || a->prob_code || a->final_obs) return false;
    const soccer_rollout_args r = run_as_rollout(*a, 1, (int64_t)h->P.n, (int64_t)h->P.n);
    return rollout_takes_swar(h, &r, nullptr);
}

static bool run_disjoint(const soccer_handle* h, const soccer_step_args& f, int64_t len, int64_t act_stride, int64_t out_stride) {
    struct Range { uintptr_t lo, hi; bool written; };
    const uint64_t n = h->P.n;
    Range r[6]; int m = 0;
    auto add = [&](const void* p, int64_t stride, size_t elem, bool written) {
        if (!p) return;
        const uintptr_t lo = reinterpret_cast<uintptr_t>(p);
        r[m++] = Range{lo, lo + (uintptr_t)(((uint64_t)(len - 1) * (uint64_t)stride + n) * elem), written};
    };
    add(f.act_a, act_stride, 1, false); add(f.act_b, act_stride, 1, false);
    add(f.obs, out_stride, 2, true); add(f.reward, out_stride, 1, true);
    add(f.terminated, out_stride, 1, true); add(f.truncated, out_stride, 1, true);
    for (int i = 0; i < m; ++i)
        for (int j = i + 1; j < m; ++j)
            if ((r[i].written || r[j].written) && r[i].lo < r[j].hi && r[j].lo < r[i].hi) return false;
    return true;
}

static bool run_extends(soccer_handle* h, const soccer_step_args* a) {
    PendingRun& R = h->run;
    const soccer_step_args& f = R.first;
    if (R.len < 1 || R.len >= (int64_t)1 << 30) return false;
    if (!a->obs != !f.obs || !a->reward != !f.reward || !a->terminated != !f.terminated || !a->truncated != !f.truncated) return false;
    const int64_t n = (int64_t)h->P.n;
    auto rows = [](const void* p, const void* q, int64_t elem) { return (int64_t)(reinterpret_cast<intptr_t>(p) - reinterpret_cast<intptr_t>(q)) / elem; };
    const int64_t da = rows(a->act_a, f.act_a, 1);
    int64_t d_out = 0;
    bool have = false, same = rows(a->act_b, f.act_b, 1) == da;
    auto out = [&](const void* p, const void* q, int64_t elem) {
        if (!q) return;
        const int64_t d = rows(p, q, elem);
        if (!have) { d_out = d; have = true; } else if (d != d_out) same = false;
    };
    out(a->obs, f.obs, 2); out(a->reward, f.reward, 1); out(a->terminated, f.terminated, 1); out(a->truncated, f.truncated, 1);
    if (!same) return false;
    int64_t as = R.act_stride, os = R.out_stride;
    if (R.len == 1) {
        as = da; os = have ? d_out : n;
        if (as < n || as % 4 != 0 || os < n || os % 4 != 0) return false;
    } else if (da != R.len * as || (have && d_out != R.len * os)) return false;
    if (!run_disjoint(h, f, R.len + 1, as, os)) return false;
    R.act_stride = as; R.out_stride = os;
    return true;
}

int flush_run(soccer_handle* h) {
    const PendingRun R = h->run;
    h->run = PendingRun{};
    if (R.len < 1) return SOCCER_OK;
    HIP_TRY(h, hipSetDevice(h->cfg.device));
    if (R.len == 1) return launch_one_step(h, &R.first);
    const soccer_rollout_args r = run_as_rollout(R.first, R.len, R.act_stride, R.out_stride);
    const soccer_rollout_shape_info keep = h->last_rollout;
    const int rc = rollout_enqueue(h, &r, nullptr, h->P.step_stats ? h->d_hist : h->d_hist_unread);
    h->last_rollout = keep;
    if (rc == SOCCER_OK) { h->capture_steps_fused += R.len; h->capture_fused_launches += 1; }
    return rc;
}

extern "C" int batched_step_ex(soccer_handle* h, const soccer_step_args* a) {
    if (!h) return fail(nullptr, SOCCER_E_INVALID, "handle is NULL");
    if (!a || (!a->act_a && !h->P.policy_a) || (!a->act_b && !h->P.policy_b))
        return fail(h, SOCCER_E_INVALID, "batched_step: an action stream is required for every player without a fixed policy");
    if (!aligned(a->u_step, 8) || !aligned(a->u_reset, 8) || !aligned(a->obs, 2) || !aligned(a->final_obs, 2) ||
        !aligned(a->reward_a_f32, 4) || !aligned(a->reward_b_f32, 4))
        return fail(h, SOCCER_E_INVALID, "batched_step: u_* must be 8-byte, reward_*_f32 4-byte and obs/final_obs 2-byte aligned");
    HIP_TRY(h, hipSetDevice(h->cfg.device));
    if (h->capturing) {
        const bool can = step_can_fuse(h, a);
        if (can && h->run.len && run_extends(h, a)) { h->run.len += 1; return SOCCER_OK; }
        if (int rc = flush_pending(h)) return rc;
        if (can) { h->run.first = *a; h->run.len = 1; return SOCCER_OK; }
    }
    return launch_one_step(h, a);
}

extern "C" int batched_step(soccer_handle* h, const int8_t* act_a, const int8_t* act_b, uint16_t* obs,
                            int8_t* reward, uint8_t* terminated, uint8_t* truncated, uint8_t* prob_code) {
    soccer_step_args a{};
    a.act_a = act_a; a.act_b = act_b; a.obs = obs; a.reward = reward;
    a.terminated = terminated; a.truncated = truncated; a.prob_code = prob_code;
    return batched_step_ex(h, &a);
}

extern "C" int soccer_exact_walk_stats(const soccer_handle* h, uint64_t* parts, uint64_t* groups) {
    if (!h) return fail(nullptr, SOCCER_E_INVALID, "handle is NULL");
    soccer_handle* hm = const_cast<soccer_handle*>(h);
    if (h->capturing) return fail(hm, SOCCER_E_STATE, "soccer_exact_walk_stats during graph capture");
    unsigned long long st[2] = {0ull, 0ull};
    if (h->d_worklist) {
        HIP_TRY(hm, hipSetDevice(h->cfg.device));
        HIP_TRY(hm, hipStreamSynchronize(h->stream));
        HIP_TRY(hm, hipMemcpy(st, worklist_count(h) + 2, sizeof st, hipMemcpyDeviceToHost));
    }
    if (parts) *parts = st[0];
    if (groups) *groups = st[1];
    return SOCCER_OK;
}
```

gym_soccer_littman94_amd/csrc/soccer_swar.hpp:

```cpp
#pragma once
#include <stdint.h>

#if defined(__HIPCC__)
#define SOCCER_HD __host__ __device__ __forceinline__
#else
#define SOCCER_HD inline
#endif

namespace soccer {
constexpr int kSlipThresholds = 40;
constexpr int kSlipStepBucketBits = 10, kSlipStepBuckets = 1 << kSlipStepBucketBits, kSlipStepCompares = 2;
constexpr int kSlipStepLdsWords = kSlipStepBuckets / 4 + 64;

namespace swar {

SOCCER_HD uint32_t perm(uint32_t hi, uint32_t lo, uint32_t sel) {
#if defined(__HIP_DEVICE_COMPILE__)
    return __builtin_amdgcn_perm(hi, lo, sel);
#else
    const uint64_t in = ((uint64_t)hi << 32) | lo;
    uint32_t r = 0;
    for (int j = 0; j < 4; ++j) {
        const uint32_t s = (sel >> (8 * j)) & 0xffu;
        uint32_t b;
        if (s >= 13u) b = 0xffu;
        else if (s == 12u) b = 0u;
        else if (s >= 8u) b = ((in >> (8 * (2 * (s - 8u) + 1) + 7)) & 1u) ? 0xffu : 0u;
        else b = (uint32_t)(in >> (8 * s)) & 0xffu;
        r |= b << (8 * j);
    }
    return r;
#endif
}
SOCCER_HD uint32_t bfi(uint32_t m, uint32_t x, uint32_t y) {
#if defined(__HIP_DEVICE_COMPILE__)
    return __builtin_amdgcn_bitop3_b32(m, x, y, 0xca);
#else
    return (m & x) | (~m & y);
#endif
}
SOCCER_HD uint32_t pk_mad(uint32_t a, uint32_t b, uint32_t c) {
#if defined(__HIP_DEVICE_COMPILE__)
    typedef unsigned short u16x2 __attribute__((ext_vector_type(2)));
    const u16x2 r = __builtin_bit_cast(u16x2, a) * __builtin_bit_cast(u16x2, b) + __builtin_bit_cast(u16x2, c);
    return __builtin_bit_cast(uint32_t, r);
#else
    const uint32_t lo = ((a & 0xffffu) * (b & 0xffffu) + (c & 0xffffu)) & 0xffffu;
    const uint32_t hi = ((a >> 16) * (b >> 16) + (c >> 16)) & 0xffffu;
    return lo | (hi << 16);
#endif
}

SOCCER_HD uint32_t pk_add(uint32_t a, uint32_t b) {
#if defined(__HIP_DEVICE_COMPILE__)
    typedef unsigned short u16x2 __attribute__((ext_vector_type(2)));
    const u16x2 r = __builtin_bit_cast(u16x2, a) + __builtin_bit_cast(u16x2, b);
    return __builtin_bit_cast(uint32_t, r);
#else
    return ((a + b) & 0xffffu) | ((((a >> 16) + (b >> 16)) & 0xffffu) << 16);
#endif
}

SOCCER_HD uint32_t rotr(uint32_t x, uint32_t r) {
#if defined(__HIP_DEVICE_COMPILE__)
    return __builtin_amdgcn_alignbit(x, x, r);
#else
    r &= 31u;
    return r ? (x >> r) | (x << (32u - r)) : x;
#endif
}

constexpr uint32_t K80 = 0x80808080u, K01 = 0x01010101u, K7F = 0x7f7f7f7fu;

SOCCER_HD uint32_t mask_of(uint32_t flag) { return perm(flag << 8, flag, 0x090b080au); }
SOCCER_HD uint32_t one_of(uint32_t flag) { return (flag >> 7) & K01; }
SOCCER_HD uint32_t is_zero(uint32_t x) { return K80 - x; }

struct Consts {
    uint32_t Wx2;
    uint32_t Wm2x2;
    uint32_t Hp1x4;
    uint32_t Wm1x4;
    uint32_t gr_lo_add;
    uint32_t gr_hi_add;
    uint32_t trunc_add;
    uint32_t obs_mul;
    uint32_t isd_ra, isd_rb, isd_p;
    uint32_t isd_ca4, isd_cb4;
    uint32_t isd_shift, isd_mask;
    uint32_t autoreset;
    uint32_t small;
    uint32_t row_lo, row_hi;
    uint32_t col_lo, col_hi;
    uint32_t grow_lo, grow_hi;
    uint32_t rew_lo, rew_hi;
    uint32_t term_lo, term_hi;
};

inline bool fits(int H, int W, int max_steps) {
    const int NI = H * (W - 2);
    return H >= 4 && W >= 7 && H * W <= 128 && 2 * NI + 2 <= 255 && max_steps >= 1 && max_steps <= 127;
}

inline Consts make_consts(int H, int W, int goal_lo, int goal_hi, int max_steps, int n_isd, const int8_t (*isd)[5],
                          bool autoreset) {
    Consts C{};
    auto splat = [](uint32_t b) { return (b & 0xffu) * K01; };
    C.Wx2 = (uint32_t)W | ((uint32_t)W << 16);
    C.Wm2x2 = (uint32_t)(W - 2) | ((uint32_t)(W - 2) << 16);
    C.Hp1x4 = splat((uint32_t)H + 1u);
    C.Wm1x4 = splat((uint32_t)W - 1u);
    C.gr_lo_add = splat(0x80u - (uint32_t)goal_lo);
    C.gr_hi_add = splat(0x7fu - (uint32_t)goal_hi);
    C.trunc_add = splat(0x80u - (uint32_t)max_steps);
    const uint32_t m = 2u * (uint32_t)(H * (W - 2) - 1);
    C.obs_mul = m | (m << 16);
    for (int k = 0; k < 4; ++k) {
        const int e = k < n_isd ? k : 0;
        C.isd_ra |= (uint32_t)(uint8_t)isd[e][0] << (8 * k);
        C.isd_rb |= (uint32_t)(uint8_t)isd[e][2] << (8 * k);
        C.isd_p |= (uint32_t)(uint8_t)isd[e][4] << (8 * k);
    }
    C.isd_ca4 = splat((uint32_t)(uint8_t)isd[0][1]);
    C.isd_cb4 = splat((uint32_t)(uint8_t)isd[0][3]);
    C.isd_shift = n_isd == 4 ? 0u : 1u;
    C.isd_mask = n_isd == 4 ? 0x03030303u : K01;
    C.autoreset = autoreset ? 1u : 0u;
    auto table = [](int n, int lo, int hi, int bias, uint32_t& tlo, uint32_t& thi) {
        uint64_t t = 0;
        for (int u = 0; u < 8; ++u) {
            int v = (u < n ? u : n - 1) - bias;
            v = v < lo ? lo : (v > hi ? hi : v);
            t |= (uint64_t)(uint8_t)v << (8 * u);
        }
        tlo = (uint32_t)t; thi = (uint32_t)(t >> 32);
    };
    C.small = (H + 2 <= 8 && W <= 8) ? 1u : 0u;
    if (C.small) {
        table(H + 2, 0, H - 1, 1, C.row_lo, C.row_hi);
        table(W, 1, W - 2, 0, C.col_lo, C.col_hi);
        auto flags = [](int n, auto f, uint32_t& tlo, uint32_t& thi) {
            uint64_t t = 0;
            for (int u = 0; u < 8 && u < n; ++u) t |= (uint64_t)(uint8_t)f(u) << (8 * u);
            tlo = (uint32_t)t; thi = (uint32_t)(t >> 32);
        };
        flags(H, [&](int r) { return r >= goal_lo && r <= goal_hi ? 0x80 : 0; }, C.grow_lo, C.grow_hi);
        flags(W, [&](int c) { return c == 0 ? 0xff : (c == W - 1 ? 0x01 : 0); }, C.rew_lo, C.rew_hi);
        flags(W, [&](int c) { return c == 0 || c == W - 1 ? 0x01 : 0; }, C.term_lo, C.term_hi);
    }
    return C;
}

struct Rand4 { uint32_t kq, rs; };

SOCCER_HD uint32_t pack_byte0(uint32_t w0, uint32_t w1, uint32_t w2, uint32_t w3) {
    return perm(perm(w3, w2, 0x0c0c0400u), perm(w1, w0, 0x0c0c0400u), 0x05040100u);
}
SOCCER_HD uint32_t pack_byte3(uint32_t w0, uint32_t w1, uint32_t w2, uint32_t w3) {
    return perm(perm(w3, w2, 0x0c0c0703u), perm(w1, w0, 0x0c0c0703u), 0x05040100u);
}
SOCCER_HD Rand4 rand_words(const uint32_t isd_shift, uint32_t w0, uint32_t w1, uint32_t w2, uint32_t w3) {
    return Rand4{pack_byte3(w0, w1, w2, w3), pack_byte0(w0, w1, w2, w3) >> isd_shift};
}
SOCCER_HD Rand4 rand_nibble(const uint32_t isd_shift, uint32_t t, uint32_t w0, uint32_t w1, uint32_t w2, uint32_t w3) {
    const uint32_t r = (4u * (t ^ 1u) + 28u) & 31u;
    const uint32_t x = pack_byte0(rotr(w0, r), rotr(w1, r), rotr(w2, r), rotr(w3, r));
    return Rand4{x, x >> (4u + isd_shift)};
}
SOCCER_HD void transpose4(uint32_t w0, uint32_t w1, uint32_t w2, uint32_t w3, uint32_t& p0, uint32_t& p1, uint32_t& p2, uint32_t& p3) {
    const uint32_t a = perm(w1, w0, 0x05010400u), b = perm(w1, w0, 0x07030602u);
    const uint32_t c = perm(w3, w2, 0x05010400u), d = perm(w3, w2, 0x07030602u);
    p0 = perm(c, a, 0x05040100u); p1 = perm(c, a, 0x07060302u); p2 = perm(d, b, 0x05040100u); p3 = perm(d, b, 0x07060302u);
}
SOCCER_HD Rand4 rand_pair(const uint32_t isd_shift, uint32_t t, uint32_t p) {
    const uint32_t sh = (t & 1u) << 2;
    return Rand4{p << sh, p >> (4u - sh + isd_shift)};
}

struct Group { uint32_t ra, ca, rb, cb, ps, tt; };

inline bool packs(int H, int W) { return H <= 8 && W <= 16; }
SOCCER_HD void unpack3(uint32_t a, uint32_t b, uint32_t t, Group& S) {
    S.ra = (a >> 4) & 0x07070707u; S.ca = a & 0x0f0f0f0fu;
    S.rb = (b >> 4) & 0x07070707u; S.cb = b & 0x0f0f0f0fu;
    S.ps = ((a >> 7) & K01) | ((b >> 6) & 0x02020202u); S.tt = t;
}
SOCCER_HD void pack3(const Group& S, uint32_t& a, uint32_t& b, uint32_t& t) {
    a = ((S.ps << 7) & K80) | (S.ra << 4) | S.ca;
    b = ((S.ps << 6) & K80) | (S.rb << 4) | S.cb;
    t = S.tt;
}

struct Out {
    uint32_t obs_lo, obs_hi;
    uint32_t fin_lo, fin_hi;
    uint32_t rew, term, trunc;
    uint32_t code;
    uint32_t finished;
    uint32_t frozen;
    uint32_t bad_action;
};

SOCCER_HD uint32_t lut8(uint32_t hi, uint32_t lo, uint32_t a) { return perm(hi, lo, a); }

constexpr uint32_t T_DR1_LO = 0x01020001u, T_DR1_HI = 0x01010101u;
constexpr uint32_t T_E_LO = 0x01000000u, T_E_HI = 0u;
constexpr uint32_t T_W_LO = 0u, T_W_HI = 0x00000001u;
constexpr uint32_t T_NZ_LO = 0x80808000u, T_NZ_HI = 0x00000080u;
constexpr uint32_t T_CANON_LO = 0x03020100u, T_CANON_HI = 0x00000004u;
SOCCER_HD uint32_t canon4(uint32_t x) { return perm(T_CANON_HI, T_CANON_LO, x & 0x07070707u); }
constexpr uint32_t T_SLIP1_LO = 0x02040300u, T_SLIP1_HI = 0x00000001u;
constexpr uint32_t T_SLIP2_LO = 0x01030400u, T_SLIP2_HI = 0x00000002u;

SOCCER_HD void move_delta(uint32_t mv, uint32_t& dr1, uint32_t& dc) {
    dr1 = lut8(T_DR1_HI, T_DR1_LO, mv);
    dc = lut8(T_E_HI, T_E_LO, mv) - lut8(T_W_HI, T_W_LO, mv);
}
template <int GEO, bool DELTAS = false>
SOCCER_HD void move4(const Consts& C, uint32_t r, uint32_t c, uint32_t mv, uint32_t dc, uint32_t score, uint32_t& nr, uint32_t& nc) {
    const uint32_t u = r + (DELTAS ? mv : lut8(T_DR1_HI, T_DR1_LO, mv));
    if (GEO == 1) {
        nr = perm(C.row_hi, C.row_lo, u);
    } else {
        const uint32_t at_top = one_of(is_zero(u));
        const uint32_t at_bot = one_of(is_zero(u ^ C.Hp1x4));
        nr = u + at_top + 0xFEFEFEFFu - at_bot;
    }
    const uint32_t ct = DELTAS ? c + dc : c + lut8(T_E_HI, T_E_LO, mv) - lut8(T_W_HI, T_W_LO, mv);
    if (GEO == 1) {
        nc = bfi(mask_of(score), ct, perm(C.col_hi, C.col_lo, ct));
    } else {
        const uint32_t edge = is_zero(ct) | is_zero(ct ^ C.Wm1x4);
        const uint32_t revert = bfi(score, 0u, edge);
        nc = bfi(mask_of(revert), c, ct);
    }
}

struct alignas(16) Quad { uint32_t x, y, z, w; };
struct SlipConsts {
    uint32_t CB[9];
    uint32_t c_off;
};
constexpr uint32_t T_VA_LO = 0x01010202u, T_VA_HI = 0x00000102u;
constexpr uint32_t T_VB_LO = 0x01020102u, T_VB_HI = 0x01020000u;
constexpr uint32_t T_CL_LO = 0x03030303u, T_CL_HI = 0x01010202u;

SOCCER_HD void slip_moves4(uint32_t c4, uint32_t aa, uint32_t ab, uint32_t& sa, uint32_t& sb, uint32_t& cls4) {
    const uint32_t sel = 0x08080808u - c4;
    const uint32_t va = perm(T_VA_HI, T_VA_LO, sel), vb = perm(T_VB_HI, T_VB_LO, sel);
    cls4 = perm(T_CL_HI, T_CL_LO, sel);
    sa = bfi(perm(0u, 0x0000ff00u, va), perm(T_SLIP1_HI, T_SLIP1_LO, aa), bfi(perm(0u, 0x00ff0000u, va), perm(T_SLIP2_HI, T_SLIP2_LO, aa), aa));
    sb = bfi(perm(0u, 0x0000ff00u, vb), perm(T_SLIP1_HI, T_SLIP1_LO, ab), bfi(perm(0u, 0x00ff0000u, vb), perm(T_SLIP2_HI, T_SLIP2_LO, ab), ab));
}

SOCCER_HD void slip_select4(const SlipConsts& L, const Quad* sub, uint32_t aa, uint32_t ab,
                            uint32_t w0, uint32_t w1, uint32_t w2, uint32_t w3,
                            uint32_t& sa, uint32_t& sb, uint32_t& k4, uint32_t& cls4) {
    const uint32_t w[4] = {w0, w1, w2, w3};
    uint32_t c4 = 0u; k4 = 0u;
#if defined(__HIP_DEVICE_COMPILE__)
#pragma unroll
#endif
    for (int j = 0; j < 4; ++j) {
        const uint32_t m = w[j] >> 2;
        uint32_t idx = 0u;
#if defined(__HIP_DEVICE_COMPILE__)
#pragma unroll
#endif
        for (int i = 0; i < 9; ++i) idx += m >= L.CB[i] ? 1u : 0u;
        const Quad th = sub[idx];
        const uint32_t q = (m >= th.y ? 1u : 0u) + (m >= th.z ? 1u : 0u) + (m >= th.w ? 1u : 0u);
        c4 |= (idx + L.c_off) << (8 * j); k4 |= q << (8 * j);
    }
    slip_moves4(c4, aa, ab, sa, sb, cls4);
}

template <int BITS = 14, int NCMP = 1>
SOCCER_HD uint32_t slip_count4_lut(const uint8_t* lut, const uint32_t* T, uint32_t w0, uint32_t w1, uint32_t w2, uint32_t w3) {
    const uint32_t w[4] = {w0, w1, w2, w3};
    uint32_t p4 = 0u;
#if defined(__HIP_DEVICE_COMPILE__)
#pragma unroll
#endif
    for (int j = 0; j < 4; ++j) {
        const uint32_t m = w[j] >> 2;
        const uint32_t below = lut[w[j] >> (32 - BITS)];
        uint32_t p = below;
#if defined(__HIP_DEVICE_COMPILE__)
#pragma unroll
#endif
        for (int c = 0; c < NCMP; ++c) p += m >= T[below + c] ? 1u : 0u;
        p4 |= p << (8 * j);
    }
    return p4;
}
SOCCER_HD void slip_from_count4(uint32_t p4, uint32_t c_off, uint32_t aa, uint32_t ab, uint32_t& sa, uint32_t& sb, uint32_t& k4, uint32_t& cls4) {
    k4 = p4 & 0x03030303u;
    slip_moves4(((p4 >> 2) & 0x3f3f3f3fu) + c_off * K01, aa, ab, sa, sb, cls4);
}
template <int BITS = 14, int NCMP = 1>
SOCCER_HD void slip_select4_lut(const uint8_t* lut, const uint32_t* T, uint32_t c_off, uint32_t aa, uint32_t ab,
                                uint32_t w0, uint32_t w1, uint32_t w2, uint32_t w3,
                                uint32_t& sa, uint32_t& sb, uint32_t& k4, uint32_t& cls4) {
    slip_from_count4(slip_count4_lut<BITS, NCMP>(lut, T, w0, w1, w2, w3), c_off, aa, ab, sa, sb, k4, cls4);
}

template <bool ZERO>
SOCCER_HD void obs4(const Consts& C, uint32_t r_a, uint32_t c_a, uint32_t r_b, uint32_t c_b, uint32_t p01, uint32_t zero7,
                    uint32_t& lo, uint32_t& hi) {
    const uint32_t jA = pk_mad(r_a, C.Wm2x2, c_a), jB = pk_mad(r_b, C.Wm2x2, c_b);
    const uint32_t gt2 = (((jB | K80) - jA) >> 6) & 0x02020202u;
    const uint32_t iA = jA - K01;
    const uint32_t q = (jB << 1) + p01 - gt2 - K01;
    lo = pk_mad(perm(0u, iA, 0x0c010c00u), C.obs_mul, perm(0u, q, 0x0c010c00u));
    hi = pk_mad(perm(0u, iA, 0x0c030c02u), C.obs_mul, perm(0u, q, 0x0c030c02u));
    if (ZERO) {
        const uint32_t z = mask_of(zero7);
        lo = bfi(perm(0u, z, 0x01010000u), 0u, lo); hi = bfi(perm(0u, z, 0x03030202u), 0u, hi);
    }
}

template <bool MASKED>
SOCCER_HD void reset4(const Consts& C, Group& S, uint32_t mask4, const Rand4& R, uint32_t& obs_lo, uint32_t& obs_hi) {
    const uint32_t idx = R.rs & C.isd_mask;
    const uint32_t ira = perm(0u, C.isd_ra, idx), irb = perm(0u, C.isd_rb, idx), ip = perm(0u, C.isd_p, idx);
    uint32_t zero7 = 0u;
    if (MASKED) {
        const uint32_t m = mask_of(((mask4 & K7F) + K7F) | mask4);
        S.ra = bfi(m, ira, S.ra); S.ca = bfi(m, C.isd_ca4, S.ca); S.rb = bfi(m, irb, S.rb); S.cb = bfi(m, C.isd_cb4, S.cb);
        S.ps = bfi(m, ip, S.ps); S.tt = bfi(m, 0u, S.tt);
        const uint32_t cc = bfi(mask_of(S.ps << 7), S.cb, S.ca);
        zero7 = is_zero(cc) | is_zero(cc ^ C.Wm1x4);
    } else {
        S.ra = ira; S.ca = C.isd_ca4; S.rb = irb; S.cb = C.isd_cb4; S.ps = ip; S.tt = 0u;
    }
    obs4<MASKED>(C, S.ra, S.ca, S.rb, S.cb, S.ps & K01, zero7, obs_lo, obs_hi);
}

struct Moves4 {
    uint32_t aa, ab;
    uint32_t sa, sb;
    uint32_t dra, dca, drb, dcb;
    uint32_t ira, irb, ip;
    uint32_t bad_action;
};
template <bool SLIP>
SOCCER_HD Moves4 step4_moves(const Consts& C, uint32_t aa_raw, uint32_t ab_raw, uint32_t sa, uint32_t sb, const Rand4& R) {
    Moves4 M;
    M.aa = canon4(aa_raw); M.ab = canon4(ab_raw); M.bad_action = (M.aa ^ aa_raw) | (M.ab ^ ab_raw);
    if (!SLIP) { M.sa = M.aa; M.sb = M.ab; } else { M.sa = sa & 0x07070707u; M.sb = sb & 0x07070707u; }
    move_delta(M.sa, M.dra, M.dca); move_delta(M.sb, M.drb, M.dcb);
    const uint32_t idx = R.rs & C.isd_mask;
    M.ira = perm(0u, C.isd_ra, idx); M.irb = perm(0u, C.isd_rb, idx); M.ip = perm(0u, C.isd_p, idx);
    return M;
}

template <bool GENERAL, bool FULL, bool SLIP, int GEO, bool TRUSTED, bool PRE>
SOCCER_HD void step4_body(const Consts& C, Group& S, uint32_t aa_raw, uint32_t ab_raw, uint32_t sa, uint32_t sb,
                          uint32_t cls4, const Rand4& R, const Moves4& M, Out& o) {
    constexpr bool TABLES = PRE && !GENERAL;
    const uint32_t ra = S.ra, ca = S.ca, rb = S.rb, cb = S.cb, ps = S.ps, t = S.tt;
    uint32_t aa = aa_raw, ab = ab_raw;
    if (PRE) { aa = M.aa; ab = M.ab; sa = M.sa; sb = M.sb; o.bad_action = M.bad_action; }
    else if (TRUSTED) o.bad_action = 0u;
    else { aa = canon4(aa_raw); ab = canon4(ab_raw); o.bad_action = (aa ^ aa_raw) | (ab ^ ab_raw); }
    const uint32_t p7 = ps << 7;
    const uint32_t pm = mask_of(p7);
    uint32_t frz7 = 0u, hold_m = 0u, frz_m = 0u;
    if (GENERAL) {
        frz7 = ps << 6;
        const uint32_t cc0 = bfi(pm, cb, ca);
        const uint32_t hold7 = frz7 | is_zero(cc0) | is_zero(cc0 ^ C.Wm1x4);
        hold_m = mask_of(hold7); frz_m = mask_of(frz7);
        aa = bfi(hold_m, 0u, aa); ab = bfi(hold_m, 0u, ab);
        if (SLIP) { sa = bfi(hold_m, 0u, sa); sb = bfi(hold_m, 0u, sb); }
    }
    if (!SLIP) { sa = aa; sb = ab; } else { sa &= 0x07070707u; sb &= 0x07070707u; }
    uint32_t gra, grb;
    if (GEO == 1) { gra = perm(C.grow_hi, C.grow_lo, ra); grb = perm(C.grow_hi, C.grow_lo, rb); }
    else { gra = bfi(ra + C.gr_hi_add, 0u, ra + C.gr_lo_add); grb = bfi(rb + C.gr_hi_add, 0u, rb + C.gr_lo_add); }
    uint32_t nra, nca, nrb, ncb;
    move4<GEO, TABLES>(C, ra, ca, TABLES ? M.dra : sa, M.dca, bfi(p7, 0u, gra), nra, nca);
    move4<GEO, TABLES>(C, rb, cb, TABLES ? M.drb : sb, M.dcb, grb & p7, nrb, ncb);
    const uint32_t A = pk_mad(ra, C.Wx2, ca), B = pk_mad(rb, C.Wx2, cb);
    const uint32_t nA = pk_mad(nra, C.Wx2, nca), nB = pk_mad(nrb, C.Wx2, ncb);
    const uint32_t e1 = is_zero(nA ^ B), e2 = is_zero(nB ^ A);
    const uint32_t sA = is_zero(nA ^ A), sB = is_zero(nB ^ B), same = is_zero(nA ^ nB);
    const uint32_t nzA = lut8(T_NZ_HI, T_NZ_LO, aa), nzB = lut8(T_NZ_HI, T_NZ_LO, ab);
    const uint32_t swap = e1 & e2;
    const uint32_t stander = bfi(nzB, 0u, e1) | bfi(nzA, 0u, e2);
    const uint32_t bounce = ((sA & nzA) & e2) | ((sB & nzB) & e1);
    const uint32_t coin = swap | bfi(stander, 0u, bounce);
    const uint32_t flip = bfi(coin, 0u, stander);
    const uint32_t cs = coin | stander;
    const uint32_t four = bfi(cs, 0u, same);
    const uint32_t mv = ~(cs | same);
    const uint32_t kb1 = R.kq, kb0c = R.kq, kb0f = R.kq << 1;
    const uint32_t amv = (four & kb1) | mv;
    const uint32_t bmv = bfi(kb1, mv, four | mv);
    const uint32_t am = mask_of(amv), bm = mask_of(bmv);
    uint32_t fra = bfi(am, nra, ra), fca = bfi(am, nca, ca), frb = bfi(bm, nrb, rb), fcb = bfi(bm, ncb, cb);
    const uint32_t p7n = bfi(coin | four, bfi(coin, kb0c, kb0f), p7 ^ flip);
    const uint32_t pmn = mask_of(p7n);
    const uint32_t cc = bfi(pmn, fcb, fca);
    uint32_t goal7, rew, term01;
    if (GEO == 1) {
        rew = perm(C.rew_hi, C.rew_lo, cc); term01 = perm(C.term_hi, C.term_lo, cc); goal7 = term01 << 7;
    } else {
        const uint32_t g0 = is_zero(cc), gW = is_zero(cc ^ C.Wm1x4);
        goal7 = g0 | gW; rew = one_of(gW) | mask_of(g0); term01 = one_of(goal7);
    }
    if (GENERAL) rew = bfi(hold_m, 0u, rew);
    uint32_t tt = t + (GENERAL ? bfi(frz_m, 0u, K01) : K01);
    const uint32_t trunc7 = tt + C.trunc_add;
    const uint32_t need7 = goal7 | trunc7;
    const uint32_t fin7 = GENERAL ? bfi(frz7, 0u, need7) : need7;
    o.rew = rew; o.term = term01; o.trunc = one_of(trunc7);
    o.finished = fin7; o.frozen = frz7 & K80;
    if (FULL) {
        uint32_t code = one_of(coin) | ((four >> 6) & 0x02020202u);
        if (SLIP) code += cls4 + (cls4 << 1);
        if (GENERAL && SLIP) code = bfi(frz_m, 0u, code);
        o.code = code;
    }
    uint32_t p01 = one_of(p7n);
    if (FULL) obs4<true>(C, fra, fca, frb, fcb, p01, goal7, o.fin_lo, o.fin_hi);
    uint32_t need_out7 = GENERAL ? (need7 | frz7) : need7;
    uint32_t obs_zero7 = goal7;
    if (!GENERAL || C.autoreset) {
        const uint32_t rm = mask_of(fin7);
        const uint32_t idx = R.rs & C.isd_mask;
        fra = bfi(rm, TABLES ? M.ira : perm(0u, C.isd_ra, idx), fra); fca = bfi(rm, C.isd_ca4, fca);
        frb = bfi(rm, TABLES ? M.irb : perm(0u, C.isd_rb, idx), frb); fcb = bfi(rm, C.isd_cb4, fcb);
        p01 = bfi(rm, TABLES ? M.ip : perm(0u, C.isd_p, idx), p01);
        tt = bfi(rm, 0u, tt);
        need_out7 = frz7;
        obs_zero7 = bfi(fin7, 0u, goal7);
    }
    obs4<GENERAL>(C, fra, fca, frb, fcb, p01, obs_zero7, o.obs_lo, o.obs_hi);
    S.ra = fra; S.ca = fca; S.rb = frb; S.cb = fcb; S.tt = tt;
    S.ps = p01 | ((need_out7 >> 6) & 0x02020202u);
}
template <bool GENERAL, bool FULL, bool SLIP, int GEO = 0, bool TRUSTED = false>
SOCCER_HD void step4(const Consts& C, Group& S, uint32_t aa_raw, uint32_t ab_raw, uint32_t sa, uint32_t sb,
                     uint32_t cls4, const Rand4& R, Out& o) {
    step4_body<GENERAL, FULL, SLIP, GEO, TRUSTED, false>(C, S, aa_raw, ab_raw, sa, sb, cls4, R, Moves4{}, o);
}
template <bool GENERAL, bool FULL, bool SLIP, int GEO = 0>
SOCCER_HD void step4_state(const Consts& C, Group& S, const Moves4& M, uint32_t cls4, const Rand4& R, Out& o) {
    step4_body<GENERAL, FULL, SLIP, GEO, false, true>(C, S, 0u, 0u, 0u, 0u, cls4, R, M, o);
}

}
}
```

Baseline: 789.8 billion.

## Drop unread statistics in fused rollouts and carry masked state across SWAR steps

Fused runs of captured steps whose statistics are never read now launch a rollout kernel variant with STATS=false, which skips the histogram accumulation and flush and removes the scratch histogram buffer. The non-general SWAR step now carries a byte-mask possession and a pre-biased truncation counter across the inner loop, so the per-step mask_of and trunc_add work is dropped. Several lookup tables are changed to return full-byte masks. Action canonicalisation is reduced to a plain mask with a cheaper bad-action test, and selected constant tables are pinned in vector registers. This adds template instantiations and register pressure, and it risks subtle semantic differences in the bad-action and obs encoding.

```diff
diff --git a/gym_soccer_littman94_amd/csrc/soccer_handle.hpp b/gym_soccer_littman94_amd/csrc/soccer_handle.hpp
--- a/gym_soccer_littman94_amd/csrc/soccer_handle.hpp
+++ b/gym_soccer_littman94_amd/csrc/soccer_handle.hpp
@@ -130,7 +130,6 @@
     bool graph_fuse = true;
     int capture_kernels = 0;
     int64_t capture_steps_fused = 0; int capture_fused_launches = 0;
-    unsigned long long* d_hist_unread = nullptr;
     int n_cu = 256;
     size_t lds_limit = 64 * 1024;
     uint4* d_sub = nullptr;
diff --git a/gym_soccer_littman94_amd/csrc/soccer_hip.hip b/gym_soccer_littman94_amd/csrc/soccer_hip.hip
--- a/gym_soccer_littman94_amd/csrc/soccer_hip.hip
+++ b/gym_soccer_littman94_amd/csrc/soccer_hip.hip
@@ -117,8 +117,6 @@
     while (h->hist_slots < (n + 255) / 256) h->hist_slots <<= 1;
     if (int rc = h->bufs.alloc(nullptr, h->hist_slots * kHistStride, &h->d_hist)) return rc;
     HIP_TRY(nullptr, hipMemset(h->d_hist, 0, sizeof(unsigned long long) * h->hist_slots * kHistStride));
-    if (int rc = h->bufs.alloc(nullptr, h->hist_slots * kHistStride, &h->d_hist_unread)) return rc;
-    HIP_TRY(nullptr, hipMemset(h->d_hist_unread, 0, sizeof(unsigned long long) * h->hist_slots * kHistStride));
     if (int rc = h->bufs.alloc_pinned(nullptr, kMappedBytes / sizeof(unsigned int), OwnedBufs::kPinnedMapped, &h->misuse_host)) return rc;
     std::memset(h->misuse_host, 0, kMappedBytes);
     HIP_TRY(nullptr, hipHostGetDevicePointer(reinterpret_cast<void**>(&h->d_misuse), h->misuse_host, 0));
diff --git a/gym_soccer_littman94_amd/csrc/soccer_rollout.hip b/gym_soccer_littman94_amd/csrc/soccer_rollout.hip
--- a/gym_soccer_littman94_amd/csrc/soccer_rollout.hip
+++ b/gym_soccer_littman94_amd/csrc/soccer_rollout.hip
@@ -93,6 +93,8 @@
     int E = h->E;
     while (E > 1 && !rollout_vec_ok(a, x, E)) E = E == 4 ? 1 : E / 2;
     const bool swar_roll = rollout_takes_swar(h, a, x);
+    if (!hist && (!swar_roll || (h->P.n & 3ull) || a->sample_actions || h->P.policy_a || h->P.policy_b || x_fin || x_code))
+        return fail(h, SOCCER_E_STATE, "rollout without statistics: not the shape of a fused run of captured steps");
     constexpr int kChunk = 4096;
     const Rules& R0 = h->rules;
     for (int s0 = 0; s0 < a->n_steps; s0 += kChunk) {
@@ -150,8 +152,10 @@
             uint64_t blocks = (groups + kBlock - 1) / kBlock;
             if (blocks > (uint64_t)h->grid_cap) blocks = h->grid_cap;
             const dim3 g((unsigned)blocks), bl(kBlock);
-#define LAUNCH_F(DV, SV, GV, FV) do { if (smem > 48 * 1024) HIP_TRY(h, hipFuncSetAttribute(reinterpret_cast<const void*>(&rollout_swar_kernel<DV, SV, GV, FV>), hipFuncAttributeMaxDynamicSharedMemorySize, (int)smem)); \
-                                      hipLaunchKernelGGL((rollout_swar_kernel<DV, SV, GV, FV>), g, bl, smem, h->stream, RS, io); } while (0)
+#define LAUNCH_T(DV, SV, GV, FV, TV) do { if (smem > 48 * 1024) HIP_TRY(h, hipFuncSetAttribute(reinterpret_cast<const void*>(&rollout_swar_kernel<DV, SV, GV, FV, TV>), hipFuncAttributeMaxDynamicSharedMemorySize, (int)smem)); \
+                                          hipLaunchKernelGGL((rollout_swar_kernel<DV, SV, GV, FV, TV>), g, bl, smem, h->stream, RS, io); } while (0)
+#define LAUNCH_F(DV, SV, GV, FV) do { if constexpr (kUnreadShape<DV, FV>) { if (!hist) LAUNCH_T(DV, SV, GV, FV, false); else LAUNCH_T(DV, SV, GV, FV, true); } \
+                                      else LAUNCH_T(DV, SV, GV, FV, true); } while (0)
 #define LAUNCH_G(DV, SV, GV) do { if (io.final_obs || io.prob_code) LAUNCH_F(DV, SV, GV, true); else LAUNCH_F(DV, SV, GV, false); } while (0)
 #define LAUNCH_S(DV, SV) do { if (h->swar_c.small) LAUNCH_G(DV, SV, 1); else LAUNCH_G(DV, SV, 0); } while (0)
             const int dm = !dyn ? 0 : (!fixed && io.sample_actions && !io.mix_a && !io.mix_b) ? 1
@@ -167,6 +171,7 @@
 #undef LAUNCH_S
 #undef LAUNCH_G
 #undef LAUNCH_F
+#undef LAUNCH_T
             }
             if (n4 < n_all) {
                 KernelParams Q = h->P;
diff --git a/gym_soccer_littman94_amd/csrc/soccer_rollout_kernels.hpp b/gym_soccer_littman94_amd/csrc/soccer_rollout_kernels.hpp
--- a/gym_soccer_littman94_amd/csrc/soccer_rollout_kernels.hpp
+++ b/gym_soccer_littman94_amd/csrc/soccer_rollout_kernels.hpp
@@ -137,7 +137,12 @@
 __device__ __forceinline__ uint32_t draw_a15(uint32_t wm) { return swar::perm(0u, wm, 0x01000100u); }
 __device__ __forceinline__ uint32_t draw_b15(uint32_t wm) { return swar::perm(0u, wm, 0x03020302u); }
 
-template <int DYNM, int SLIPM, bool GENERAL, int GEO, bool FULL = false>
+template <int DYNM, bool FULL> constexpr bool kUnreadShape = DYNM == 0 && !FULL;
+template <int DYNM, int SLIPM, bool GENERAL, int GEO, bool FULL, bool STATS>
+constexpr bool kHoistTables = GEO == 1 && !GENERAL && !(DYNM == 1 && SLIPM == 0 && !FULL) &&
+                              !((DYNM == 4 || DYNM == 5) && SLIPM == 1 && FULL);
+
+template <int DYNM, int SLIPM, bool GENERAL, int GEO, bool FULL = false, bool STATS = true>
 __device__ __forceinline__ void rollout_swar_group(const RolloutSwar& R, const RolloutIO& IO, const SlipSrc& slip,
                                                    const uint2* mix_a_in, const uint2* mix_b_in, const int8_t* pol_a_in, const int8_t* pol_b_in,
                                                    uint32_t* act_lds,
@@ -189,7 +194,13 @@
         const uint32_t cc0 = swar::bfi(swar::mask_of(S.ps << 7), S.cb, S.ca);
         swar::obs4<true>(R.C, S.ra, S.ca, S.rb, S.cb, S.ps & swar::K01, swar::is_zero(cc0) | swar::is_zero(cc0 ^ R.C.Wm1x4), s_lo, s_hi);
     }
-    const swar::Consts& C = R.C;
+    swar::Consts Cv = R.C;
+    if (kHoistTables<DYNM, SLIPM, GENERAL, GEO, FULL, STATS>) {
+        asm volatile("" : "+v"(Cv.row_lo), "+v"(Cv.col_lo), "+v"(Cv.grow_lo), "+v"(Cv.rew_lo), "+v"(Cv.term_lo));
+    }
+    const swar::Consts& C = Cv;
+    swar::Carry4 K{};
+    if (!GENERAL) K = swar::carry_of(C, S);
     const unsigned long long q = (R.lane_offset + i0) >> 2;
     uint32_t fin_loc = 0u, nz_loc = 0u, neg_loc = 0u;
     uint32_t p0 = 0u, p1 = 0u, p2 = 0u, p3 = 0u;
@@ -251,7 +262,7 @@
         if (SLIP) {
             const Philox4 blk = philox4x32_10((uint32_t)q, (uint32_t)(q >> 32), (uint32_t)tick, (uint32_t)(tick >> 32), R.key0, R.key1);
             uint32_t k4 = 0u;
-            const uint32_t ca4 = TRUSTED ? a4 : swar::canon4(a4), cb4 = TRUSTED ? b4 : swar::canon4(b4);
+            const uint32_t ca4 = TRUSTED ? a4 : a4 & 0x07070707u, cb4 = TRUSTED ? b4 : b4 & 0x07070707u;
             if (SLIPM == 2) swar::slip_select4_lut(slip.lut, slip.T, R.L.c_off, ca4, cb4, blk.w[0], blk.w[1], blk.w[2], blk.w[3], sa, sb, k4, cls4);
             else swar::slip_select4(R.L, slip.sub, ca4, cb4, blk.w[0], blk.w[1], blk.w[2], blk.w[3], sa, sb, k4, cls4);
             rnd = swar::Rand4{k4 << 6, swar::pack_byte0(blk.w[0], blk.w[1], blk.w[2], blk.w[3]) >> C.isd_shift};
@@ -265,7 +276,8 @@
             rnd = swar::rand_pair(C.isd_shift, t, p0);
             if (t & 1u) { asm volatile(""); p0 = p1; p1 = p2; p2 = p3; }
         }
-        swar::step4<GENERAL, FULL, SLIP, GEO, TRUSTED>(C, S, a4, b4, sa, sb, cls4, rnd, o);
+        if constexpr (GENERAL) swar::step4<true, FULL, SLIP, GEO, TRUSTED>(C, S, a4, b4, sa, sb, cls4, rnd, o);
+        else swar::step4_carry<FULL, SLIP, GEO, TRUSTED>(C, K, a4, b4, sa, sb, cls4, rnd, o);
         s_lo = o.obs_lo; s_hi = o.obs_hi;
         const long long row = (long long)s * IO.out_stride;
         uint32_t j0 = i0; asm volatile("" : "+v"(j0));
@@ -279,9 +291,9 @@
                                                           reinterpret_cast<unsigned long long*>(reinterpret_cast<uint8_t*>(IO.final_obs + row) + (j0 << 1)));
             if (IO.prob_code) __builtin_nontemporal_store(o.code, reinterpret_cast<uint32_t*>(reinterpret_cast<uint8_t*>(IO.prob_code + row) + j0));
         }
-        fin_loc += (uint32_t)__builtin_popcount(o.finished & swar::K80);
-        if (GENERAL) { nz_loc += (uint32_t)__builtin_popcount(o.rew & swar::K01); neg_loc += (uint32_t)__builtin_popcount(o.rew & swar::K80); }
-        else {
+        if (STATS) fin_loc += (uint32_t)__builtin_popcount(o.finished & swar::K80);
+        if (STATS && GENERAL) { nz_loc += (uint32_t)__builtin_popcount(o.rew & swar::K01); neg_loc += (uint32_t)__builtin_popcount(o.rew & swar::K80); }
+        else if (STATS) {
             nz_loc += (uint32_t)__builtin_popcount(o.term); neg_loc += (uint32_t)__builtin_popcount(o.rew);
         }
         if (lane_acc) {
@@ -294,16 +306,18 @@
         if (!TRUSTED) bad_any |= o.bad_action;
         if (!STAGED) { aa = naa; ab = nab; }
     }
+    if (!GENERAL) S = swar::group_of(C, K);
     fin_tot += fin_loc; nz_tot += nz_loc;
     neg_tot += GENERAL ? neg_loc : (neg_loc - nz_loc) / 7u;
 }
 
-template <int DYNM, int SLIPM, int GEO = 0, bool FULL = false>
+template <int DYNM, int SLIPM, int GEO = 0, bool FULL = false, bool STATS = true>
 __global__ __launch_bounds__(kBlock) void rollout_swar_kernel(const RolloutSwar R, const RolloutIO IO) {
     constexpr bool SLIP = SLIPM != 0;
     constexpr bool DYN = DYNM >= 2;
     extern __shared__ __attribute__((aligned(16))) uint32_t smem[];
-    HistAcc<false> hist; hist.init_at(R.hist, R.hist_mask);
+    static_assert(STATS || kUnreadShape<DYNM, FULL>, "only a fused run of captured steps goes without statistics");
+    HistAcc<false> hist; if (STATS) hist.init_at(R.hist, R.hist_mask);
     SlipSrc slip{R.sub, nullptr, nullptr};
     const uint2* mix_a = reinterpret_cast<const uint2*>(IO.mix_a);
     const uint2* mix_b = reinterpret_cast<const uint2*>(IO.mix_b);
@@ -353,8 +367,8 @@
         uint32_t acc[4] = {0u, 0u, 0u, 0u};
         const uint32_t edge = swar::is_zero(S.ca) | swar::is_zero(S.cb) | swar::is_zero(S.ca ^ R.C.Wm1x4) | swar::is_zero(S.cb ^ R.C.Wm1x4);
         const bool special = R.C.autoreset == 0u || (((S.ps << 6) | edge) & swar::K80) != 0u;
-        if (special) rollout_swar_group<DYNM, SLIPM, true, GEO, FULL>(R, IO, slip, mix_a, mix_b, pol_a, pol_b, act_lds, i0, tick0, S, fin_tot, nz_tot, neg_tot, acc, frozen_any, bad_any);
-        else rollout_swar_group<DYNM, SLIPM, false, GEO, FULL>(R, IO, slip, mix_a, mix_b, pol_a, pol_b, act_lds, i0, tick0, S, fin_tot, nz_tot, neg_tot, acc, frozen_any, bad_any);
+        if (special) rollout_swar_group<DYNM, SLIPM, true, GEO, FULL, STATS>(R, IO, slip, mix_a, mix_b, pol_a, pol_b, act_lds, i0, tick0, S, fin_tot, nz_tot, neg_tot, acc, frozen_any, bad_any);
+        else rollout_swar_group<DYNM, SLIPM, false, GEO, FULL, STATS>(R, IO, slip, mix_a, mix_b, pol_a, pol_b, act_lds, i0, tick0, S, fin_tot, nz_tot, neg_tot, acc, frozen_any, bad_any);
         uint8_t* sw = R.state + i0;
         if (R.layout == kStatePacked) {
             uint32_t pa, pb, pt;
@@ -365,7 +379,7 @@
         *reinterpret_cast<uint32_t*>(sw + 2 * R.state_stride) = S.rb; *reinterpret_cast<uint32_t*>(sw + 3 * R.state_stride) = S.cb;
         *reinterpret_cast<uint32_t*>(sw + 4 * R.state_stride) = S.ps; *reinterpret_cast<uint32_t*>(sw + 5 * R.state_stride) = S.tt;
         }
-        hist.add_totals(fin_tot, (int32_t)nz_tot - 2 * (int32_t)neg_tot, nz_tot);
+        if (STATS) hist.add_totals(fin_tot, (int32_t)nz_tot - 2 * (int32_t)neg_tot, nz_tot);
         if (IO.return_sum != nullptr || IO.episode_count != nullptr) {
             int32_t ret[4] = {(int32_t)(int16_t)(acc[0] & 0xffffu), (int32_t)(int16_t)(acc[0] >> 16), (int32_t)(int16_t)(acc[1] & 0xffffu), (int32_t)(int16_t)(acc[1] >> 16)};
             int32_t eps[4] = {(int32_t)(acc[2] & 0xffffu), (int32_t)(acc[2] >> 16), (int32_t)(acc[3] & 0xffffu), (int32_t)(acc[3] >> 16)};
@@ -375,7 +389,7 @@
     }
     if (frozen_any) R.misuse[0] = 1u;
     if (bad_any) R.misuse[1] = 1u;
-    hist.flush_at(R.hist, R.hist_mask);
-}
-
-}
+    if (STATS) hist.flush_at(R.hist, R.hist_mask);
+}
+
+}
diff --git a/gym_soccer_littman94_amd/csrc/soccer_step.hip b/gym_soccer_littman94_amd/csrc/soccer_step.hip
--- a/gym_soccer_littman94_amd/csrc/soccer_step.hip
+++ b/gym_soccer_littman94_amd/csrc/soccer_step.hip
@@ -181,7 +181,7 @@
     if (R.len == 1) return launch_one_step(h, &R.first);
     const soccer_rollout_args r = run_as_rollout(R.first, R.len, R.act_stride, R.out_stride);
     const soccer_rollout_shape_info keep = h->last_rollout;
-    const int rc = rollout_enqueue(h, &r, nullptr, h->P.step_stats ? h->d_hist : h->d_hist_unread);
+    const int rc = rollout_enqueue(h, &r, nullptr, h->P.step_stats ? h->d_hist : nullptr);
     h->last_rollout = keep;
     if (rc == SOCCER_OK) { h->capture_steps_fused += R.len; h->capture_fused_launches += 1; }
     return rc;
diff --git a/gym_soccer_littman94_amd/csrc/soccer_swar.hpp b/gym_soccer_littman94_amd/csrc/soccer_swar.hpp
--- a/gym_soccer_littman94_amd/csrc/soccer_swar.hpp
+++ b/gym_soccer_littman94_amd/csrc/soccer_swar.hpp
@@ -119,7 +119,7 @@
         const int e = k < n_isd ? k : 0;
         C.isd_ra |= (uint32_t)(uint8_t)isd[e][0] << (8 * k);
         C.isd_rb |= (uint32_t)(uint8_t)isd[e][2] << (8 * k);
-        C.isd_p |= (uint32_t)(uint8_t)isd[e][4] << (8 * k);
+        C.isd_p |= (isd[e][4] ? 0xffu : 0u) << (8 * k);
     }
     C.isd_ca4 = splat((uint32_t)(uint8_t)isd[0][1]);
     C.isd_cb4 = splat((uint32_t)(uint8_t)isd[0][3]);
@@ -144,7 +144,7 @@
             for (int u = 0; u < 8 && u < n; ++u) t |= (uint64_t)(uint8_t)f(u) << (8 * u);
             tlo = (uint32_t)t; thi = (uint32_t)(t >> 32);
         };
-        flags(H, [&](int r) { return r >= goal_lo && r <= goal_hi ? 0x80 : 0; }, C.grow_lo, C.grow_hi);
+        flags(H, [&](int r) { return r >= goal_lo && r <= goal_hi ? 0xff : 0; }, C.grow_lo, C.grow_hi);
         flags(W, [&](int c) { return c == 0 ? 0xff : (c == W - 1 ? 0x01 : 0); }, C.rew_lo, C.rew_hi);
         flags(W, [&](int c) { return c == 0 || c == W - 1 ? 0x01 : 0; }, C.term_lo, C.term_hi);
     }
@@ -206,9 +206,13 @@
 constexpr uint32_t T_DR1_LO = 0x01020001u, T_DR1_HI = 0x01010101u;
 constexpr uint32_t T_E_LO = 0x01000000u, T_E_HI = 0u;
 constexpr uint32_t T_W_LO = 0u, T_W_HI = 0x00000001u;
-constexpr uint32_t T_NZ_LO = 0x80808000u, T_NZ_HI = 0x00000080u;
+constexpr uint32_t T_DC1_LO = 0x02010101u, T_DC1_HI = 0x01010100u;
+constexpr uint32_t T_NZ_LO = 0x80808000u, T_NZ_HI = 0x01010180u;
 constexpr uint32_t T_CANON_LO = 0x03020100u, T_CANON_HI = 0x00000004u;
 SOCCER_HD uint32_t canon4(uint32_t x) { return perm(T_CANON_HI, T_CANON_LO, x & 0x07070707u); }
+SOCCER_HD uint32_t bad_actions4(uint32_t a_raw, uint32_t b_raw, uint32_t nz_a, uint32_t nz_b) {
+    return ((nz_a | nz_b) & K01) | ((a_raw | b_raw) & 0xf8f8f8f8u);
+}
 constexpr uint32_t T_SLIP1_LO = 0x02040300u, T_SLIP1_HI = 0x00000001u;
 constexpr uint32_t T_SLIP2_LO = 0x01030400u, T_SLIP2_HI = 0x00000002u;
 
@@ -226,9 +230,9 @@
         const uint32_t at_bot = one_of(is_zero(u ^ C.Hp1x4));
         nr = u + at_top + 0xFEFEFEFFu - at_bot;
     }
-    const uint32_t ct = DELTAS ? c + dc : c + lut8(T_E_HI, T_E_LO, mv) - lut8(T_W_HI, T_W_LO, mv);
+    const uint32_t ct = DELTAS ? c + dc : c + lut8(T_DC1_HI, T_DC1_LO, mv) + 0xFEFEFEFFu;
     if (GEO == 1) {
-        nc = bfi(mask_of(score), ct, perm(C.col_hi, C.col_lo, ct));
+        nc = bfi(score, ct, perm(C.col_hi, C.col_lo, ct));
     } else {
         const uint32_t edge = is_zero(ct) | is_zero(ct ^ C.Wm1x4);
         const uint32_t revert = bfi(score, 0u, edge);
@@ -309,9 +313,9 @@
 SOCCER_HD void obs4(const Consts& C, uint32_t r_a, uint32_t c_a, uint32_t r_b, uint32_t c_b, uint32_t p01, uint32_t zero7,
                     uint32_t& lo, uint32_t& hi) {
     const uint32_t jA = pk_mad(r_a, C.Wm2x2, c_a), jB = pk_mad(r_b, C.Wm2x2, c_b);
-    const uint32_t gt2 = (((jB | K80) - jA) >> 6) & 0x02020202u;
+    const uint32_t nge2 = (((jA | K80) - jB) >> 6) & 0x02020202u;
     const uint32_t iA = jA - K01;
-    const uint32_t q = (jB << 1) + p01 - gt2 - K01;
+    const uint32_t q = ((jB << 1) + p01) + nge2 + 0xFCFCFCFDu;
     lo = pk_mad(perm(0u, iA, 0x0c010c00u), C.obs_mul, perm(0u, q, 0x0c010c00u));
     hi = pk_mad(perm(0u, iA, 0x0c030c02u), C.obs_mul, perm(0u, q, 0x0c030c02u));
     if (ZERO) {
@@ -323,7 +327,7 @@
 template <bool MASKED>
 SOCCER_HD void reset4(const Consts& C, Group& S, uint32_t mask4, const Rand4& R, uint32_t& obs_lo, uint32_t& obs_hi) {
     const uint32_t idx = R.rs & C.isd_mask;
-    const uint32_t ira = perm(0u, C.isd_ra, idx), irb = perm(0u, C.isd_rb, idx), ip = perm(0u, C.isd_p, idx);
+    const uint32_t ira = perm(0u, C.isd_ra, idx), irb = perm(0u, C.isd_rb, idx), ip = perm(0u, C.isd_p, idx) & K01;
     uint32_t zero7 = 0u;
     if (MASKED) {
         const uint32_t m = mask_of(((mask4 & K7F) + K7F) | mask4);
@@ -355,17 +359,18 @@
     return M;
 }
 
-template <bool GENERAL, bool FULL, bool SLIP, int GEO, bool TRUSTED, bool PRE>
+template <bool GENERAL, bool FULL, bool SLIP, int GEO, bool TRUSTED, bool PRE, bool CARRY = false>
 SOCCER_HD void step4_body(const Consts& C, Group& S, uint32_t aa_raw, uint32_t ab_raw, uint32_t sa, uint32_t sb,
                           uint32_t cls4, const Rand4& R, const Moves4& M, Out& o) {
+    static_assert(!(CARRY && GENERAL), "the step form has no room for the needs_reset bit");
     constexpr bool TABLES = PRE && !GENERAL;
     const uint32_t ra = S.ra, ca = S.ca, rb = S.rb, cb = S.cb, ps = S.ps, t = S.tt;
     uint32_t aa = aa_raw, ab = ab_raw;
-    if (PRE) { aa = M.aa; ab = M.ab; sa = M.sa; sb = M.sb; o.bad_action = M.bad_action; }
-    else if (TRUSTED) o.bad_action = 0u;
-    else { aa = canon4(aa_raw); ab = canon4(ab_raw); o.bad_action = (aa ^ aa_raw) | (ab ^ ab_raw); }
-    const uint32_t p7 = ps << 7;
-    const uint32_t pm = mask_of(p7);
+    if (PRE) { aa = M.aa; ab = M.ab; sa = M.sa; sb = M.sb; }
+    else if (!TRUSTED) { aa = aa_raw & 0x07070707u; ab = ab_raw & 0x07070707u; }
+    uint32_t nzA = lut8(T_NZ_HI, T_NZ_LO, aa), nzB = lut8(T_NZ_HI, T_NZ_LO, ab);
+    o.bad_action = PRE ? M.bad_action : TRUSTED ? 0u : bad_actions4(aa_raw, ab_raw, nzA, nzB);
+    const uint32_t pm = CARRY ? ps : mask_of(ps << 7);
     uint32_t frz7 = 0u, hold_m = 0u, frz_m = 0u;
     if (GENERAL) {
         frz7 = ps << 6;
@@ -373,6 +378,7 @@
         const uint32_t hold7 = frz7 | is_zero(cc0) | is_zero(cc0 ^ C.Wm1x4);
         hold_m = mask_of(hold7); frz_m = mask_of(frz7);
         aa = bfi(hold_m, 0u, aa); ab = bfi(hold_m, 0u, ab);
+        nzA = bfi(hold_m, 0u, nzA); nzB = bfi(hold_m, 0u, nzB);
         if (SLIP) { sa = bfi(hold_m, 0u, sa); sb = bfi(hold_m, 0u, sb); }
     }
     if (!SLIP) { sa = aa; sb = ab; } else { sa &= 0x07070707u; sb &= 0x07070707u; }
@@ -380,13 +386,12 @@
     if (GEO == 1) { gra = perm(C.grow_hi, C.grow_lo, ra); grb = perm(C.grow_hi, C.grow_lo, rb); }
     else { gra = bfi(ra + C.gr_hi_add, 0u, ra + C.gr_lo_add); grb = bfi(rb + C.gr_hi_add, 0u, rb + C.gr_lo_add); }
     uint32_t nra, nca, nrb, ncb;
-    move4<GEO, TABLES>(C, ra, ca, TABLES ? M.dra : sa, M.dca, bfi(p7, 0u, gra), nra, nca);
-    move4<GEO, TABLES>(C, rb, cb, TABLES ? M.drb : sb, M.dcb, grb & p7, nrb, ncb);
+    move4<GEO, TABLES>(C, ra, ca, TABLES ? M.dra : sa, M.dca, bfi(pm, 0u, gra), nra, nca);
+    move4<GEO, TABLES>(C, rb, cb, TABLES ? M.drb : sb, M.dcb, grb & pm, nrb, ncb);
     const uint32_t A = pk_mad(ra, C.Wx2, ca), B = pk_mad(rb, C.Wx2, cb);
     const uint32_t nA = pk_mad(nra, C.Wx2, nca), nB = pk_mad(nrb, C.Wx2, ncb);
     const uint32_t e1 = is_zero(nA ^ B), e2 = is_zero(nB ^ A);
     const uint32_t sA = is_zero(nA ^ A), sB = is_zero(nB ^ B), same = is_zero(nA ^ nB);
-    const uint32_t nzA = lut8(T_NZ_HI, T_NZ_LO, aa), nzB = lut8(T_NZ_HI, T_NZ_LO, ab);
     const uint32_t swap = e1 & e2;
     const uint32_t stander = bfi(nzB, 0u, e1) | bfi(nzA, 0u, e2);
     const uint32_t bounce = ((sA & nzA) & e2) | ((sB & nzB) & e1);
@@ -400,7 +405,7 @@
     const uint32_t bmv = bfi(kb1, mv, four | mv);
     const uint32_t am = mask_of(amv), bm = mask_of(bmv);
     uint32_t fra = bfi(am, nra, ra), fca = bfi(am, nca, ca), frb = bfi(bm, nrb, rb), fcb = bfi(bm, ncb, cb);
-    const uint32_t p7n = bfi(coin | four, bfi(coin, kb0c, kb0f), p7 ^ flip);
+    const uint32_t p7n = bfi(coin | four, bfi(coin, kb0c, kb0f), pm ^ flip);
     const uint32_t pmn = mask_of(p7n);
     const uint32_t cc = bfi(pmn, fcb, fca);
     uint32_t goal7, rew, term01;
@@ -412,7 +417,7 @@
     }
     if (GENERAL) rew = bfi(hold_m, 0u, rew);
     uint32_t tt = t + (GENERAL ? bfi(frz_m, 0u, K01) : K01);
-    const uint32_t trunc7 = tt + C.trunc_add;
+    const uint32_t trunc7 = CARRY ? tt : tt + C.trunc_add;
     const uint32_t need7 = goal7 | trunc7;
     const uint32_t fin7 = GENERAL ? bfi(frz7, 0u, need7) : need7;
     o.rew = rew; o.term = term01; o.trunc = one_of(trunc7);
@@ -423,8 +428,8 @@
         if (GENERAL && SLIP) code = bfi(frz_m, 0u, code);
         o.code = code;
     }
-    uint32_t p01 = one_of(p7n);
-    if (FULL) obs4<true>(C, fra, fca, frb, fcb, p01, goal7, o.fin_lo, o.fin_hi);
+    uint32_t pmo = pmn;
+    if (FULL) obs4<true>(C, fra, fca, frb, fcb, pmn & K01, goal7, o.fin_lo, o.fin_hi);
     uint32_t need_out7 = GENERAL ? (need7 | frz7) : need7;
     uint32_t obs_zero7 = goal7;
     if (!GENERAL || C.autoreset) {
@@ -432,20 +437,36 @@
         const uint32_t idx = R.rs & C.isd_mask;
         fra = bfi(rm, TABLES ? M.ira : perm(0u, C.isd_ra, idx), fra); fca = bfi(rm, C.isd_ca4, fca);
         frb = bfi(rm, TABLES ? M.irb : perm(0u, C.isd_rb, idx), frb); fcb = bfi(rm, C.isd_cb4, fcb);
-        p01 = bfi(rm, TABLES ? M.ip : perm(0u, C.isd_p, idx), p01);
-        tt = bfi(rm, 0u, tt);
+        pmo = bfi(rm, TABLES ? M.ip : perm(0u, C.isd_p, idx), pmn);
+        tt = bfi(rm, CARRY ? C.trunc_add : 0u, tt);
         need_out7 = frz7;
         obs_zero7 = bfi(fin7, 0u, goal7);
     }
+    const uint32_t p01 = pmo & K01;
     obs4<GENERAL>(C, fra, fca, frb, fcb, p01, obs_zero7, o.obs_lo, o.obs_hi);
     S.ra = fra; S.ca = fca; S.rb = frb; S.cb = fcb; S.tt = tt;
-    S.ps = p01 | ((need_out7 >> 6) & 0x02020202u);
+    S.ps = CARRY ? pmo : p01 | ((need_out7 >> 6) & 0x02020202u);
 }
 template <bool GENERAL, bool FULL, bool SLIP, int GEO = 0, bool TRUSTED = false>
 SOCCER_HD void step4(const Consts& C, Group& S, uint32_t aa_raw, uint32_t ab_raw, uint32_t sa, uint32_t sb,
                      uint32_t cls4, const Rand4& R, Out& o) {
     step4_body<GENERAL, FULL, SLIP, GEO, TRUSTED, false>(C, S, aa_raw, ab_raw, sa, sb, cls4, R, Moves4{}, o);
 }
+
+struct Carry4 { uint32_t ra, ca, rb, cb, pm, tb; };
+SOCCER_HD Carry4 carry_of(const Consts& C, const Group& S) {
+    return Carry4{S.ra, S.ca, S.rb, S.cb, mask_of(S.ps << 7), S.tt + C.trunc_add};
+}
+SOCCER_HD Group group_of(const Consts& C, const Carry4& K) {
+    return Group{K.ra, K.ca, K.rb, K.cb, K.pm & K01, K.tb - C.trunc_add};
+}
+template <bool FULL, bool SLIP, int GEO = 0, bool TRUSTED = false>
+SOCCER_HD void step4_carry(const Consts& C, Carry4& K, uint32_t aa_raw, uint32_t ab_raw, uint32_t sa, uint32_t sb,
+                           uint32_t cls4, const Rand4& R, Out& o) {
+    Group S{K.ra, K.ca, K.rb, K.cb, K.pm, K.tb};
+    step4_body<false, FULL, SLIP, GEO, TRUSTED, false, true>(C, S, aa_raw, ab_raw, sa, sb, cls4, R, Moves4{}, o);
+    K = Carry4{S.ra, S.ca, S.rb, S.cb, S.ps, S.tt};
+}
 template <bool GENERAL, bool FULL, bool SLIP, int GEO = 0>
 SOCCER_HD void step4_state(const Consts& C, Group& S, const Moves4& M, uint32_t cls4, const Rand4& R, Out& o) {
     step4_body<GENERAL, FULL, SLIP, GEO, false, true>(C, S, 0u, 0u, 0u, 0u, cls4, R, M, o);
```

Result: faster. 807.7 billion (median of 6 runs) (+2.3%).
